# AlessioSam/LADiff

Hardware: AMD Instinct MI355X
Metric: motions/sec (196-frame, 50-step DDIM, bs128) (higher is better)
Workload: dtype f16x3+f32; 1 GPU; headline:ddim50_cfg7.5_b128_f196_c263_humanml3d; prompts_per_gpu=128, global_batch=128, frames=196, scheduler=ddim, denoising_steps=50, parallelism=dp1, loop=persistent pipeline kernel (16-row blocks x 86)

## Files before the change

### include/ladiff_hip_debug.h

```cpp
#ifndef LADIFF_HIP_DEBUG_H
#define LADIFF_HIP_DEBUG_H

#include "ladiff_hip.h"

#ifdef __cplusplus
extern "C" {
#endif

LADIFF_API int ladiff_debug_set_stage_waves(int waves_per_simd);
LADIFF_API int ladiff_debug_set_handoff(int tagged);
LADIFF_API int ladiff_debug_set_stage_plan(int v);
LADIFF_API int ladiff_debug_set_poll_pause(int mask, int len);
LADIFF_API int ladiff_debug_set_stage_delay(int mask, int len);
LADIFF_API int ladiff_debug_set_pacing(int eighths, int mask);
LADIFF_API int ladiff_debug_set_xcd_local(int on);
LADIFF_API int ladiff_debug_set_decoder_fusion(int on);
LADIFF_API int ladiff_debug_set_mlp_variant(int v);

LADIFF_API int ladiff_debug_set_loop_thresholds(int look_ahead_from, int small_upto);
LADIFF_API int ladiff_debug_set_graph_epoch_rule(int on);
LADIFF_API int ladiff_debug_graph_instantiations(void);

#ifdef LADIFF_STAMPS
LADIFF_API void ladiff_debug_set_stamps(unsigned long long* p);
LADIFF_API void ladiff_debug_set_sys_stamps(unsigned long long* p);
LADIFF_API void ladiff_debug_set_probe(int v);
#endif

#ifdef __cplusplus
}
#endif
#endif
```

### ladiff_amd/_lib.py

```python
import ctypes
import os
from ctypes import c_char_p, c_double, c_float, c_int, c_size_t, c_uint64, c_void_p

import numpy as np
import torch

_HERE = os.path.dirname(os.path.abspath(__file__))
LIB_PATH = os.path.join(_HERE, "libladiff_hip.so")

MAX_LATENTS = 8
MAX_FRAMES = 224
COEF_STRIDE = 8
COEF_K_NOISE, COEF_K_M = 5, 6
ACT = {"none": 0, "relu": 1, "gelu": 2, "silu": 3, "qgelu": 4, "lrelu": 5}


class LadiffHipError(RuntimeError):
    pass


SPLIT_MODES = ("f16x3", "bf16x3", "split")


def is_split(precision):
# ... 69 lines not shown
    "ladiff_reverse_status_offset_bytes": (c_size_t, [c_int, c_int, c_int, c_int]),
    "ladiff_debug_set_stage_plan": (c_int, [c_int]),
    "ladiff_debug_set_poll_pause": (c_int, [c_int, c_int]),
    "ladiff_debug_set_stage_delay": (c_int, [c_int, c_int]),
    "ladiff_debug_set_pacing": (c_int, [c_int, c_int]),
    "ladiff_debug_set_loop_thresholds": (c_int, [c_int, c_int]),
    "ladiff_debug_set_graph_epoch_rule": (c_int, [c_int]),
    "ladiff_debug_graph_instantiations": (c_int, []),
    "ladiff_sampler_set_fault": (c_int, [c_void_p, c_int, c_int]),
    "ladiff_sampler_set_noise_generator": (c_int, [c_void_p, c_uint64, ctypes.c_uint32, c_int]),
    "ladiff_noise_fill": (c_int, [c_uint64, ctypes.c_uint32, c_int, c_int, c_int, c_int, c_void_p, c_void_p]),
    "ladiff_reverse_workspace_bytes": (c_size_t, [c_int, c_int, c_int, c_int]),
    "ladiff_diffusion_reverse": (c_int, [c_void_p, c_void_p, c_void_p, c_uint64, c_void_p, c_void_p, c_void_p, c_void_p, c_void_p,
                                         c_void_p, c_void_p, c_void_p, c_float, c_float, c_int, c_int, c_int, c_int, c_int,
                                         c_void_p, c_void_p, c_size_t, c_int, c_void_p]),
    "ladiff_diffusion_reverse_prompts": (c_int, [c_void_p, c_void_p, c_void_p, c_uint64, c_void_p, c_void_p, c_void_p, c_void_p, c_void_p,
                                                 c_void_p, c_void_p, c_void_p, c_float, c_float, c_int, c_int, c_int, c_int, c_int,
                                                 c_void_p, c_void_p, c_size_t, c_int, c_void_p, c_void_p, c_void_p, c_int, c_void_p]),
    "ladiff_diffusion_reverse_multistep": (c_int, [c_void_p, c_void_p, c_void_p, c_uint64, c_void_p, c_void_p, c_void_p, c_void_p, c_void_p,
                                                   c_void_p, c_void_p, c_void_p, c_float, c_float, c_int, c_int, c_int, c_int, c_int,
                                                   c_void_p, c_void_p, c_size_t, c_int, c_void_p, c_void_p, c_void_p, c_int, c_void_p,
                                                   c_void_p]),
    "ladiff_diffusion_reverse_from": (c_int, [c_void_p, c_void_p, c_void_p, c_uint64, c_void_p, c_void_p, c_void_p, c_void_p, c_void_p,
                                              c_void_p, c_void_p, c_void_p, c_float, c_float, c_int, c_int, c_int, c_int, c_int,
                                              c_void_p, c_void_p, c_size_t, c_int, c_void_p, c_void_p, c_void_p, c_int, c_void_p,
                                              c_void_p, c_void_p, c_int, c_void_p]),
    "ladiff_diffusion_reverse_record": (c_int, [c_void_p, c_void_p, c_void_p, c_uint64, c_void_p, c_void_p, c_void_p, c_void_p, c_void_p,
                                                c_void_p, c_void_p, c_void_p, c_float, c_float, c_int, c_int, c_int, c_int, c_int,
                                                c_void_p, c_void_p, c_size_t, c_int, c_void_p, c_void_p, c_void_p, c_int, c_void_p,
                                                c_void_p, c_void_p, c_int, c_void_p, c_void_p, c_void_p]),
    "ladiff_noise_fill_prompts": (c_int, [c_void_p, c_void_p, c_int, c_int, c_int, c_int, c_void_p, c_void_p]),
    "ladiff_encoder_num_params": (c_int, []),
    "ladiff_encoder_param_name": (c_char_p, [c_int]),
    "ladiff_encoder_workspace_bytes": (c_size_t, [c_int, c_int, c_int, c_int]),
    "ladiff_vae_encode": (c_int, [c_void_p, c_void_p, c_void_p, c_void_p, c_void_p, c_void_p, c_int, c_int, c_int, c_int,
                                  c_void_p, c_void_p, c_void_p, c_void_p, c_size_t, c_void_p]),
    "ladiff_vae_encode_dvae": (c_int, [c_void_p, c_void_p, c_void_p, c_void_p, c_void_p, c_void_p, c_int, c_int, c_int, c_int,
                                       c_void_p, c_void_p, c_void_p, c_void_p, c_size_t, c_void_p, c_void_p, c_int, c_void_p]),
    "ladiff_vae_losses_workspace_bytes": (c_size_t, [c_int, c_int, c_int, c_int, c_int]),
    "ladiff_vae_losses": (c_int, [c_void_p, c_void_p, c_void_p, c_void_p, c_void_p, c_void_p, c_int, c_int, c_int, c_int, c_int,
                                  c_double, c_double, c_double, c_void_p, c_void_p, c_void_p, c_size_t, c_void_p]),
    "ladiff_denoiser_forward_timesteps_workspace_bytes": (c_size_t, [c_int, c_int]),
    "ladiff_denoiser_forward_timesteps": (c_int, [c_void_p, c_void_p, c_void_p, c_int, c_void_p, c_void_p, c_int, c_int, c_void_p, c_void_p,
                                                  c_void_p, c_size_t, c_void_p]),
    "ladiff_q_sample": (c_int, [c_void_p, c_void_p, c_void_p, c_int, c_void_p, c_int, c_uint64, ctypes.c_uint32, c_void_p, c_void_p, c_int,
                                c_int, c_void_p]),
    "ladiff_diffusion_losses_workspace_bytes": (c_size_t, [ctypes.c_int64]),
    "ladiff_diffusion_losses": (c_int, [c_void_p, c_void_p, ctypes.c_int64, c_double, c_void_p, c_void_p, c_void_p, c_size_t, c_void_p]),
    "ladiff_clip_num_params": (c_int, []),
    "ladiff_clip_param_name": (c_char_p, [c_int]),
    "ladiff_clip_workspace_bytes": (c_size_t, [c_int, c_int]),
    "ladiff_clip_text_encode": (c_int, [c_void_p, c_void_p, c_int, c_int, c_void_p, c_int, c_int, c_int, c_void_p, c_void_p,
                                        c_size_t, c_void_p]),
    "ladiff_clip_workspace_bytes_ragged": (c_size_t, [c_int, c_int]),
    "ladiff_clip_text_encode_ragged": (c_int, [c_void_p, c_void_p, c_int, c_int, c_void_p, c_int, c_int, c_int, c_void_p, c_void_p,
                                               c_void_p, c_int, c_void_p, c_void_p, c_size_t, c_void_p]),
    "ladiff_t2m_movement_num_params": (c_int, []),
    "ladiff_t2m_movement_param_name": (c_char_p, [c_int]),
    "ladiff_t2m_motion_num_params": (c_int, []),
    "ladiff_t2m_motion_param_name": (c_char_p, [c_int]),
    "ladiff_t2m_text_num_params": (c_int, []),
    "ladiff_t2m_text_param_name": (c_char_p, [c_int]),
    "ladiff_t2m_movement_workspace_bytes": (c_size_t, [c_int, c_int, c_int]),
    "ladiff_t2m_motion_workspace_bytes": (c_size_t, [c_int, c_int]),
    "ladiff_t2m_text_workspace_bytes": (c_size_t, [c_int, c_int]),
    "ladiff_t2m_movement_encode": (c_int, [c_void_p, c_void_p, c_int, c_int, c_int, c_int, c_void_p, c_void_p, c_size_t,
                                           c_void_p]),
    "ladiff_t2m_motion_encode": (c_int, [c_void_p, c_void_p, c_void_p, c_int, c_int, c_void_p, c_void_p, c_size_t, c_void_p]),
    "ladiff_t2m_text_encode": (c_int, [c_void_p, c_void_p, c_void_p, c_void_p, c_int, c_int, c_void_p, c_void_p, c_size_t,
                                       c_void_p]),
    "ladiff_feats2joints": (c_int, [c_void_p, c_void_p, c_void_p, c_int, c_int, c_int, c_int, c_void_p, c_void_p]),
    "ladiff_joints2feats": (c_int, [c_void_p, c_void_p, c_int, c_int, c_int, c_void_p, c_float, c_void_p, c_void_p, c_void_p, c_void_p]),
    "ladiff_joint_ape_ave": (c_int, [c_void_p, c_void_p, c_void_p, c_void_p, c_int, c_int, c_int, c_void_p, c_float, c_void_p, c_void_p,
                                     c_void_p]),
    "ladiff_joint_mr": (c_int, [c_void_p, c_void_p, c_void_p, c_int, c_int, c_int, c_void_p, c_void_p, c_void_p]),
    "ladiff_decoder_workspace_bytes": (c_size_t, [c_int, c_int, c_int, c_int]),
    "ladiff_vae_decode": (c_int, [c_void_p, c_void_p, c_void_p, c_void_p, c_void_p, c_int, c_int, c_int, c_int, c_void_p,
                                  c_void_p, c_size_t, c_void_p]),
    "ladiff_debug_set_stage_waves": (c_int, [c_int]),
    "ladiff_debug_set_handoff": (c_int, [c_int]),
    "ladiff_debug_set_xcd_local": (c_int, [c_int]),
    "ladiff_debug_set_decoder_fusion": (c_int, [c_int]),
    "ladiff_debug_set_mlp_variant": (c_int, [c_int]),
    "ladiff_reverse_plan": (c_int, [c_int, c_int, c_void_p, c_int, c_int, c_int, c_int, c_void_p, c_void_p]),
    "ladiff_decoder_graph_create": (c_int, [ctypes.POINTER(c_void_p)]),
    "ladiff_decoder_graph_destroy": (c_int, [c_void_p]),
    "ladiff_vae_decode_graphed": (c_int, [c_void_p, c_void_p, c_void_p, c_uint64, c_void_p, c_void_p, c_void_p, c_void_p, c_int, c_int, c_int,
                                          c_int, c_int, c_void_p, c_void_p, c_size_t, c_void_p]),
    "ladiff_vae_decode_ragged": (c_int, [c_void_p, c_void_p, c_void_p, c_void_p, c_void_p, c_void_p, c_int, c_int, c_int, c_int,
                                         c_int, c_void_p, c_void_p, c_size_t, c_void_p]),
    "ladiff_vae_decode_att_maps": (c_int, [c_void_p, c_void_p, c_void_p, c_void_p, c_void_p, c_void_p, c_int, c_int, c_int, c_int,
                                           c_int, c_void_p, c_void_p, c_void_p, c_size_t, c_void_p]),
}

EXPORTS = tuple(_SIGNATURES)
_lib = None
LIB_PATH_BF16 = os.path.join(_HERE, "libladiff_hip_bf16.so")


def select_split_format(fmt):
    global LIB_PATH, _lib
    if fmt not in ("fp16", "bf16"):
        raise ValueError(f'split format must be "fp16" or "bf16", got {fmt!r}')
    path = LIB_PATH_BF16 if fmt == "bf16" else os.path.join(_HERE, "libladiff_hip.so")
    if _lib is not None and path != LIB_PATH:
        raise LadiffHipError("select_split_format() after the library has been used: weight tables of the other format exist")
    LIB_PATH = path


def lib():
    global _lib
    if _lib is None:
        if not os.path.exists(LIB_PATH):
            raise LadiffHipError(f"{LIB_PATH} not found: build it with `python -m ladiff_amd.build` "
                                 "(the HIP library is the only implementation of this path; there is no CPU fallback)")
        cdll = ctypes.CDLL(LIB_PATH)
        for name, (res, args) in _SIGNATURES.items():
            fn = getattr(cdll, name)
            fn.restype, fn.argtypes = res, args
        _lib = cdll
    return _lib


def check(rc):
    if rc != 0:
        raise LadiffHipError(f"libladiff_hip: {lib().ladiff_error_string(rc).decode()} (code {rc})")


def ptr(t, dtype=torch.float32):
    if t is None:
        return None
    if not t.is_cuda:
        raise LadiffHipError("libladiff_hip works on GPU tensors only; got a CPU tensor (no CPU fallback exists)")
    if t.dtype != dtype:
        raise LadiffHipError(f"expected {dtype}, got {t.dtype}")
    if not t.is_contiguous():
        raise LadiffHipError("expected a contiguous tensor")
    return t.data_ptr()


def stream_ptr():
    return torch.cuda.current_stream().cuda_stream


def param_names(kind):
    l = lib()
    n = getattr(l, f"ladiff_{kind}_num_params")()
    return [getattr(l, f"ladiff_{kind}_param_name")(i).decode() for i in range(n)]


class WeightTable:
    _next_generation = 1

    def __init__(self, kind, tensors, n_names=None, no_split=(), pad_rows=None):
        self.generation = WeightTable._next_generation
        WeightTable._next_generation += 1
        names = param_names(kind)
        if n_names is not None:
            names = names[:n_names]
        self.no_split = set(no_split)
        self.pad_rows = dict(pad_rows or {})
        self.names = names
        self.tensors = []
        for n in names:
            if n not in tensors:
                raise LadiffHipError(f"missing weight {n}")
# ... 107 lines not shown
```

### ladiff_amd/csrc/api.hip

```cpp
#include <algorithm>
#include <cstdlib>
#include <cstring>
#include <vector>

#include "model.h"
#include "sampler.h"
#include "../../include/ladiff_hip_debug.h"

using namespace ladiff;

namespace {

inline hipStream_t S(ladiff_stream_t s) { return reinterpret_cast<hipStream_t>(s); }

bool all_set(const float* const* w, size_t n) {
    if (w == nullptr) return false;
    for (size_t i = 0; i < n; ++i)
        if (w[i] == nullptr) return false;
    return true;
}
template <class W>
bool load_weights(W& dst, const float* const* ptrs) {
    if (!all_set(ptrs, sizeof(W) / sizeof(const float*))) return false;
    std::memcpy(&dst, ptrs, sizeof(W));
// ... 206 lines not shown
}
int ladiff_init_latents(const float* noise, const int32_t* counts, float sigma, float* latents, int B, int T,
                        ladiff_stream_t stream) {
    LADIFF_CHECK_ARG(noise && latents && B > 0 && T > 0);
    return launch_init_latents(noise, counts, sigma, latents, B, T, S(stream));
}
int ladiff_init_latents_from(const float* z0, const float* noise, const uint64_t* seeds, const uint32_t* prompt_index, const int32_t* counts,
                             const float* coef, const int32_t* starts, int first_step, float* latents, int B, int T, ladiff_stream_t stream) {
    LADIFF_CHECK_ARG(z0 && coef && latents && B > 0 && T > 0 && first_step >= 0);
    LADIFF_CHECK_ARG(noise != nullptr || seeds != nullptr);
    LADIFF_CHECK_ARG(prompt_index == nullptr || seeds != nullptr);
    if ((reinterpret_cast<uintptr_t>(z0) & 15) || (reinterpret_cast<uintptr_t>(noise) & 15) || (reinterpret_cast<uintptr_t>(latents) & 15) ||
        (reinterpret_cast<uintptr_t>(seeds) & 7) || (reinterpret_cast<uintptr_t>(prompt_index) & 3) || (reinterpret_cast<uintptr_t>(starts) & 3))
        return LADIFF_ERR_SHAPE;
    const NoiseGen gen = noise == nullptr ? NoiseGen{0u, 0u, 0u, 1, reinterpret_cast<const unsigned long long*>(seeds), prompt_index}
                                          : NoiseGen{0u, 0u, 0u, 0};
    return launch_init_latents_from(z0, noise, gen, counts, coef, starts, first_step, latents, B, T, nullptr, S(stream));
}
int ladiff_finalize_latents(const float* latents, const int32_t* counts, float* z, int B, int T, ladiff_stream_t stream) {
    LADIFF_CHECK_ARG(latents && z && B > 0 && T > 0);
    return launch_finalize_latents(latents, counts, z, B, T, S(stream));
}

int ladiff_sampler_create(void** sampler) {
    LADIFF_CHECK_ARG(sampler);
    *sampler = new Sampler();
    return 0;
}
int ladiff_sampler_destroy(void* sampler) {
    Sampler* sp = reinterpret_cast<Sampler*>(sampler);
    if (sp == nullptr) return 0;
    (void)hipDeviceSynchronize();
    sp->drain_retired();
    if (sp->exec) (void)hipGraphExecDestroy(sp->exec);
    if (sp->setup) (void)hipGraphExecDestroy(sp->setup);
    if (sp->ev0) (void)hipEventDestroy(sp->ev0);
    if (sp->ev1) (void)hipEventDestroy(sp->ev1);
    for (hipEvent_t e : sp->wev) (void)hipEventDestroy(e);
    sp->cap.destroy();
    delete sp;
    return 0;
}

int ladiff_reverse_plan(int B, int T, const int32_t* h_counts, int masked, int loop_mode, int f16x3, int cfg, int* rows_per_block, int* n_blocks) {
    LADIFF_CHECK_ARG(B >= 1 && T >= 1 && T <= LADIFF_MAX_LATENTS && loop_mode >= 1 && loop_mode <= 3 && rows_per_block && n_blocks);
    if (!cfg && masked && h_counts == nullptr) return LADIFF_ERR_UNSUPPORTED;
    std::vector<unsigned char> plan;
    int mr = 2, nb = 0;
    choose_plan(B, T, h_counts, masked != 0, loop_mode, f16x3 != 0, plan, &mr, &nb, cfg != 0);
    *rows_per_block = 16 * mr; *n_blocks = nb;
    return 0;
}

int ladiff_debug_set_stage_waves(int waves_per_simd) {
    LADIFF_CHECK_ARG(waves_per_simd == 1 || waves_per_simd == 2);
    g_loop.waves16 = waves_per_simd;
    return 0;
}

int ladiff_debug_set_handoff(int tagged) {
    LADIFF_CHECK_ARG(tagged == 0 || tagged == 1);
    g_loop.handoff = tagged;
    return 0;
}

int ladiff_debug_set_mlp_variant(int v) {
#ifdef LADIFF_STAMPS
    LADIFF_CHECK_ARG((v >= 0 && v <= 3) || (v >= 11 && v <= 17) || (v >= 21 && v <= 26));
#else
    LADIFF_CHECK_ARG(v >= 0 && v <= 3);
#endif
    g_dec.mlp_variant = v;
    return 0;
}

int ladiff_debug_set_decoder_fusion(int on) {
    LADIFF_CHECK_ARG(on >= 0 && on <= 254 && (on & 3) != 3 && (on & 48) != 48);
    g_dec.post_off = (on & 128) ? 1 : 0;
    g_dec.out_cross = (on & 64) ? 0 : 1;
    g_dec.fused_mlp = on & 3;
    g_dec.small_rows_path = (on & 4) ? 0 : 1;
    g_dec.final_split = (on & 8) ? 0 : 1;
    g_dec.fused_attn = (on & 16) ? 0 : (on & 32) ? 2 : 1;
    return 0;
}

int ladiff_debug_set_stage_plan(int v) {
    LADIFF_CHECK_ARG(v >= 0 && v <= 1);
    g_loop.stage_plan = v;
    return 0;
}

int ladiff_debug_set_poll_pause(int mask, int len) {
    LADIFF_CHECK_ARG(mask >= 0 && mask <= 255 && len >= 0 && len <= 64);
    g_loop.poll_pause = mask | (len << 8);
    return 0;
}

int ladiff_debug_set_pacing(int eighths, int mask) {
    if (eighths == -1) { g_loop.pace = -1; return 0; }
    LADIFF_CHECK_ARG(eighths >= 0 && eighths <= 8 && mask >= 0 && mask <= 255);
    g_loop.pace = eighths | (mask << 8);
    return 0;
}

int ladiff_debug_set_stage_delay(int mask, int len) {
    LADIFF_CHECK_ARG(mask >= -1 && mask <= 255 && len >= 0 && len <= 64);
    g_loop.stage_delay = mask < 0 ? -1 : (mask | (len << 8));
    return 0;
}

int ladiff_debug_set_loop_thresholds(int look_ahead_from, int small_upto) {
    LADIFF_CHECK_ARG(look_ahead_from >= -1 && small_upto >= -1);
    g_loop.look_ahead_from = look_ahead_from;
    g_loop.small_upto = small_upto;
    return 0;
}

int ladiff_debug_set_graph_epoch_rule(int on) {
    LADIFF_CHECK_ARG(on == 0 || on == 1);
    g_graph_epoch_rule = on;
    return 0;
}

int ladiff_debug_graph_instantiations(void) { return g_graph_instantiations.load(); }

int ladiff_debug_set_xcd_local(int on) {
    LADIFF_CHECK_ARG(on >= 0 && on <= 2);
    g_loop.xcd_local = on;
    return 0;
}

int ladiff_sampler_set_loop(void* sampler, int mode) {
    Sampler* sp = reinterpret_cast<Sampler*>(sampler);
    LADIFF_CHECK_ARG(sp != nullptr && mode >= 0 && mode <= 3);
    sp->loop = mode != 0;
    sp->loop_mode = mode;
    return 0;
}

int ladiff_sampler_loop_ms(void* sampler, float* ms) {
    Sampler* sp = reinterpret_cast<Sampler*>(sampler);
    LADIFF_CHECK_ARG(sp != nullptr && ms != nullptr && sp->ev1 != nullptr);
    LADIFF_HIP(hipEventSynchronize(sp->ev1));
    LADIFF_HIP(hipEventElapsedTime(ms, sp->ev0, sp->ev1));
    return 0;
}

int ladiff_sampler_set_window_timing(void* sampler, int on) {
    Sampler* sp = reinterpret_cast<Sampler*>(sampler);
    LADIFF_CHECK_ARG(sp != nullptr);
    sp->time_windows = on != 0;
    return 0;
}

int ladiff_sampler_window_ms(void* sampler, float* loop_ms_sum, int* n_windows) {
    Sampler* sp = reinterpret_cast<Sampler*>(sampler);
    LADIFF_CHECK_ARG(sp != nullptr && loop_ms_sum != nullptr && n_windows != nullptr);
    float sum = 0.f;
    for (int i = 0; i < sp->n_windows; ++i) {
        float ms = 0.f;
        LADIFF_HIP(hipEventSynchronize(sp->wev[2 * i + 1]));
        LADIFF_HIP(hipEventElapsedTime(&ms, sp->wev[2 * i], sp->wev[2 * i + 1]));
        sum += ms;
    }
    *loop_ms_sum = sum; *n_windows = sp->n_windows;
// ... 476 lines not shown
```

### ladiff_amd/csrc/attention.hip

```cpp
#include "kernels.h"

namespace ladiff {

constexpr int SA_FMAX = LADIFF_MAX_FRAMES;
constexpr int SA_NKT = SA_FMAX / 32;

struct AttnGeom { int nheads, ld, koff, voff, out_ld, causal; };

__global__ __launch_bounds__(256) void dec_self_attn_kernel(const float* __restrict__ qkv, const int32_t* __restrict__ lengths,
                                                            const uint32_t* __restrict__ keybits, float* __restrict__ out,
                                                            int B, int F, int split_out, const AttnGeom g,
                                                            const int32_t* __restrict__ row_off, int shared_qkv) {
    __shared__ __attribute__((aligned(16))) float Ks[SA_FMAX * DH];
    __shared__ __attribute__((aligned(16))) float Vs[SA_FMAX * DH];
    const int tid = threadIdx.x, lane = tid & 63, wave = tid >> 6;
    const int b = blockIdx.y / g.nheads, h = blockIdx.y % g.nheads;
    int len = F;
    uint32_t kb[SA_NKT + 1];
    if (keybits != nullptr) {
        len = 1;
#pragma unroll
        for (int i = 0; i < SA_NKT; ++i) {
            kb[i] = keybits[(size_t)b * 8 + i];
            if (kb[i]) len = 32 * i + 32 - __builtin_clz(kb[i]);
// ... 46 lines not shown
            f32x16 acc;
#pragma unroll
            for (int i = 0; i < 16; ++i) acc[i] = 0.f;
            const int r = kt * 32 + q;
#pragma unroll
            for (int g8 = 0; g8 < 8; ++g8) {
                const f32x4 a = ld4(Ks + r * DH + ((((g8 << 1) + h2) ^ (r & 15)) << 2));
#pragma unroll
                for (int e = 0; e < 4; ++e) acc = __builtin_amdgcn_mfma_f32_32x32x2f32(a[e], qf[g8][e], acc, 0, 0, 0);
            }
#pragma unroll
            for (int i = 0; i < 16; ++i) {
                const int kin = (i & 3) + 8 * (i >> 2) + 4 * h2;
                const bool ok = ((kb[kt] >> kin) & 1u) && (!g.causal || kt * 32 + kin <= qrow);
                const float s = ok ? acc[i] : -INFINITY;
                acc[i] = s;
                m = fmaxf(m, s);
            }
            sT[kt] = acc;
        }
    }
    m = fmaxf(m, __shfl_xor(m, 32, 64));

    float l = 0.f;
#pragma unroll
    for (int kt = 0; kt < SA_NKT; ++kt) {
        if (kt < nkt) {
#pragma unroll
            for (int i = 0; i < 16; ++i) {
                const float pv = expf(sT[kt][i] - m);
                sT[kt][i] = pv;
                l += pv;
            }
        }
    }
    l += __shfl_xor(l, 32, 64);

    f32x16 o0, o1;
#pragma unroll
    for (int i = 0; i < 16; ++i) { o0[i] = 0.f; o1[i] = 0.f; }
#pragma unroll
    for (int kt = 0; kt < SA_NKT; ++kt) {
        if (kt < nkt) {
#pragma unroll
            for (int i = 0; i < 16; ++i) {
                const int key = kt * 32 + (i & 3) + 8 * (i >> 2) + 4 * h2;
                const float a0 = Vs[key * DH + q];
                const float a1 = Vs[key * DH + 32 + q];
                o0 = __builtin_amdgcn_mfma_f32_32x32x2f32(a0, sT[kt][i], o0, 0, 0, 0);
                o1 = __builtin_amdgcn_mfma_f32_32x32x2f32(a1, sT[kt][i], o1, 0, 0, 0);
            }
        }
    }

    if (qrow < F) {
        const float inv = 1.f / l;
        float* rowp = out + (row0 + qrow) * g.out_ld;
        const int c0 = h * DH + 4 * h2;
#pragma unroll
        for (int rg = 0; rg < 4; ++rg) {
            f32x4 v0, v1;
#pragma unroll
            for (int e = 0; e < 4; ++e) { v0[e] = o0[4 * rg + e] * inv; v1[e] = o1[4 * rg + e] * inv; }
            if (split_out) {
                store_split4(rowp, c0 + 8 * rg, v0);
                store_split4(rowp, c0 + 32 + 8 * rg, v1);
            } else {
                st4(rowp + c0 + 8 * rg, v0);
                st4(rowp + c0 + 32 + 8 * rg, v1);
            }
        }
    }
}


__device__ __forceinline__ void split8(const float (&v)[8], s16x8& hi, s16x8& lo) {
    split8(f32x4{v[0], v[1], v[2], v[3]}, f32x4{v[4], v[5], v[6], v[7]}, hi, lo);
}

template <int FM, int NT>
__global__ __launch_bounds__(NT, NT == 64 ? 2 : 1) void self_attn_split_kernel(const float* __restrict__ qkv, const int32_t* __restrict__ lengths,
                                                               const uint32_t* __restrict__ keybits, float* __restrict__ out,
                                                               int B, int F, int split_out, const AttnGeom g,
                                                               const int32_t* __restrict__ row_off, int shared_qkv) {
    constexpr int NKT = FM / 32, IT = FM * 16 / NT, VLD = FM + 8;
    static_assert(FM % 32 == 0 && (FM * 16) % NT == 0 && NT % 64 == 0 && (FM / 4) % (NT / 64) == 0 && NT / 64 >= FM / 32, "a wave per query tile");
    __shared__ __attribute__((aligned(16))) s16 Kp[2 * FM * DH];
    __shared__ __attribute__((aligned(16))) s16 Vt[2 * DH * VLD];
    s16* const Kh = Kp; s16* const Kl = Kp + FM * DH;
    s16* const Vth = Vt; s16* const Vtl = Vt + DH * VLD;
    float* const Vtmp = reinterpret_cast<float*>(Kp);
    const int tid = threadIdx.x, lane = tid & 63, wave = tid >> 6;
    const int b = blockIdx.x / g.nheads, h = blockIdx.x % g.nheads;
    int len = F;
    uint32_t kb[NKT + 1];
    if (keybits != nullptr) {
        len = 1;
#pragma unroll
        for (int i = 0; i < NKT; ++i) {
            kb[i] = keybits[(size_t)b * 8 + i];
            if (kb[i]) len = 32 * i + 32 - __builtin_clz(kb[i]);
        }
        len = len > F ? F : len;
    } else {
        len = lengths != nullptr ? lengths[b] : F;
        len = len < 1 ? 1 : (len > F ? F : len);
#pragma unroll
        for (int i = 0; i < NKT; ++i) kb[i] = len >= 32 * i + 32 ? 0xFFFFFFFFu : (len > 32 * i ? (1u << (len - 32 * i)) - 1u : 0u);
    }
    const int nkt = (len + 31) >> 5;
    size_t row0 = (size_t)b * F;
    if (row_off != nullptr) { row0 = row_off[b]; F = row_off[b + 1] - row_off[b]; }
    const size_t base = (shared_qkv ? (size_t)0 : row0) * g.ld + h * DH;

    const int qt = wave;
    const int q = lane & 31, h2 = lane >> 5;
    const int qrow = qt * 32 + q;

    s16x8 qh[4], ql[4];
#pragma unroll
    for (int ks = 0; ks < 4; ++ks) {
        float v[8] = {0.f, 0.f, 0.f, 0.f, 0.f, 0.f, 0.f, 0.f};
        if (qrow < F) {
            const f32x4 a = ld4(qkv + base + (size_t)qrow * g.ld + 16 * ks + 8 * h2);
            const f32x4 c = ld4(qkv + base + (size_t)qrow * g.ld + 16 * ks + 8 * h2 + 4);
#pragma unroll
            for (int e = 0; e < 4; ++e) { v[e] = a[e] * (0.125f * 1.4426950408889634f); v[4 + e] = c[e] * (0.125f * 1.4426950408889634f); }
        }
        split8(v, qh[ks], ql[ks]);
    }


    f32x4 kk[IT], vv[IT];
#pragma unroll
    for (int it = 0; it < IT; ++it) {
        const int id = tid + it * NT, r = id >> 4, c = id & 15;
        kk[it] = f32x4{0.f, 0.f, 0.f, 0.f}; vv[it] = kk[it];
        if (r < nkt * 32 && r < F) {
            const float* src = qkv + base + (size_t)r * g.ld + c * 4;
            kk[it] = ld4(src + g.koff);
            vv[it] = ld4(src + g.voff);
        }
    }
#pragma unroll
    for (int it = 0; it < IT; ++it) {
        const int id = tid + it * NT, r = id >> 4, c = id & 15;
        if (r < nkt * 32) st4(Vtmp + r * DH + c * 4, vv[it]);
    }
    __syncthreads();
    {
        const int d = tid & 63, kg = tid >> 6;
        for (int p = 0; p < FM / 4 / (NT / 64); ++p) {
            const int k0 = (p * (NT / 64) + kg) * 4;
            if (k0 < nkt * 32) {
                s16x4 hi, lo;
                split4(Vtmp[k0 * DH + d], Vtmp[(k0 + 1) * DH + d], Vtmp[(k0 + 2) * DH + d], Vtmp[(k0 + 3) * DH + d], hi, lo);
                *reinterpret_cast<s16x4*>(Vth + d * VLD + k0) = hi;
                *reinterpret_cast<s16x4*>(Vtl + d * VLD + k0) = lo;
            }
        }
    }
    __syncthreads();
#pragma unroll
    for (int it = 0; it < IT; ++it) {
        const int id = tid + it * NT, r = id >> 4, c = id & 15;
        if (r < nkt * 32) {
            s16x4 hi, lo;
            split4(kk[it], hi, lo);
            const int off = r * DH + ((((c >> 1) ^ ((r >> 1) & 7)) << 3) | ((c & 1) << 2));
            *reinterpret_cast<s16x4*>(Kh + off) = hi;
            *reinterpret_cast<s16x4*>(Kl + off) = lo;
        }
    }
    __syncthreads();

    if (qt * 32 >= F) return;
// ... 19 lines not shown
            if (kb[kt] == 0xFFFFFFFFu && !g.causal) {
#pragma unroll
                for (int i = 0; i < 16; ++i) m = fmaxf(m, acc[i]);
            } else {
#pragma unroll
                for (int i = 0; i < 16; ++i) {
                    const int kin = (i & 3) + 8 * (i >> 2) + 4 * h2;
                    const bool ok = ((kb[kt] >> kin) & 1u) && (!g.causal || kt * 32 + kin <= qrow);
                    const float s = ok ? acc[i] : -INFINITY;
                    acc[i] = s;
                    m = fmaxf(m, s);
                }
            }
            sT[kt] = acc;
        }
    }
    m = fmaxf(m, __shfl_xor(m, 32, 64));

    float l = 0.f;
#pragma unroll
    for (int kt = 0; kt < NKT; ++kt) {
        if (kt < nkt) {
#pragma unroll
            for (int i = 0; i < 16; ++i) {
                const float pv = __builtin_amdgcn_exp2f(sT[kt][i] - m);
                sT[kt][i] = pv;
                l += pv;
            }
        }
    }
    l += __shfl_xor(l, 32, 64);

    f32x16 o0, o1;
#pragma unroll
    for (int i = 0; i < 16; ++i) { o0[i] = 0.f; o1[i] = 0.f; }
#pragma unroll
    for (int kt = 0; kt < NKT; ++kt) {
        if (kt < nkt) {
#pragma unroll
            for (int mm = 0; mm < 2; ++mm) {
                float pv[8];
#pragma unroll
                for (int j = 0; j < 8; ++j) pv[j] = sT[kt][8 * mm + j];
                s16x8 ph, pl;
                split8(pv, ph, pl);
                const int k1 = 32 * kt + 16 * mm + 4 * h2;
#pragma unroll
                for (int t = 0; t < 2; ++t) {
                    const int voff = (32 * t + q) * VLD + k1;
                    const s16x4 h_a = *reinterpret_cast<const s16x4*>(Vth + voff), h_b = *reinterpret_cast<const s16x4*>(Vth + voff + 8);
                    const s16x4 l_a = *reinterpret_cast<const s16x4*>(Vtl + voff), l_b = *reinterpret_cast<const s16x4*>(Vtl + voff + 8);
                    const s16x8 vh = {h_a[0], h_a[1], h_a[2], h_a[3], h_b[0], h_b[1], h_b[2], h_b[3]};
                    const s16x8 vl = {l_a[0], l_a[1], l_a[2], l_a[3], l_b[0], l_b[1], l_b[2], l_b[3]};
                    f32x16& o = t == 0 ? o0 : o1;
                    o = MFMA32_S16(vl, ph, o, 0, 0, 0);
                    o = MFMA32_S16(vh, pl, o, 0, 0, 0);
                    o = MFMA32_S16(vh, ph, o, 0, 0, 0);
                }
            }
        }
    }

    if (qrow < F) {
        const float inv = 1.f / l;
        float* rowp = out + (row0 + qrow) * g.out_ld;
        const int c0 = h * DH + 4 * h2;
#pragma unroll
        for (int rg = 0; rg < 4; ++rg) {
            f32x4 v0, v1;
#pragma unroll
            for (int e = 0; e < 4; ++e) { v0[e] = o0[4 * rg + e] * inv; v1[e] = o1[4 * rg + e] * inv; }
            if (split_out) {
                store_split4(rowp, c0 + 8 * rg, v0);
                store_split4(rowp, c0 + 32 + 8 * rg, v1);
            } else {
                st4(rowp + c0 + 8 * rg, v0);
                st4(rowp + c0 + 32 + 8 * rg, v1);
            }
        }
    }
}

int launch_self_attention_split(const float* qkv, const int32_t* lengths, const uint32_t* keybits, float* out, int B, int F,
                                 int nheads, int causal, int split_out, hipStream_t s, const int32_t* row_off, int shared_qkv) {
    if (F > SA_FMAX || F < 1 || nheads < 1) return LADIFF_ERR_SHAPE;
    if (B == 0) return 0;
    const int W = nheads * DH;
    const AttnGeom g{nheads, 3 * W, W, 2 * W, W, causal};
    if (F <= 32) hipLaunchKernelGGL((self_attn_split_kernel<32, 64>), dim3(B * nheads), dim3(64), 0, s, qkv, lengths, keybits, out, B, F, split_out, g, row_off, shared_qkv);
    else hipLaunchKernelGGL((self_attn_split_kernel<SA_FMAX, 512>), dim3(B * nheads), dim3(512), 0, s, qkv, lengths, keybits, out, B, F, split_out, g, row_off, shared_qkv);
    LADIFF_LAUNCH_CHECK();
    return 0;
}

int launch_self_attention(const float* qkv, const int32_t* lengths, const uint32_t* keybits, float* out, int B, int F, int nheads,
                          int causal, int split_out, hipStream_t s, const int32_t* row_off) {
    if (F > SA_FMAX || F < 1 || nheads < 1) return LADIFF_ERR_SHAPE;
    if (B == 0) return 0;
    const int W = nheads * DH;
    const AttnGeom g{nheads, 3 * W, W, 2 * W, W, causal};
    const int nqt = (F + 31) / 32;
    hipLaunchKernelGGL(dec_self_attn_kernel, dim3((nqt + 3) / 4, B * nheads), dim3(256), 0, s, qkv, lengths, keybits, out, B, F,
                       split_out, g, row_off, 0);
    LADIFF_LAUNCH_CHECK();
    return 0;
}

int launch_decoder_self_attention(const float* qkv, const int32_t* lengths, const uint32_t* keybits, float* out, int B, int F,
                                  int split_out, hipStream_t s, const int32_t* row_off, int shared_qkv) {
    if (F > SA_FMAX || F < 1) return LADIFF_ERR_SHAPE;
    if (lengths == nullptr && keybits == nullptr) return LADIFF_ERR_ARG;
    if (B == 0) return 0;
    const AttnGeom g{H, 3 * D, D, 2 * D, D, 0};
    const int nqt = (F + 31) / 32;
    hipLaunchKernelGGL(dec_self_attn_kernel, dim3((nqt + 3) / 4, B * H), dim3(256), 0, s, qkv, lengths, keybits, out, B, F,
                       split_out, g, row_off, shared_qkv);
    LADIFF_LAUNCH_CHECK();
    return 0;
}

template <int T>
__global__ __launch_bounds__(256) void dec_cross_attn_kernel(const float* __restrict__ q, const float* __restrict__ kv,
                                                             const int32_t* __restrict__ counts, float* __restrict__ out,
                                                             int B, int F, int M, int split_out) {
    const int row = blockIdx.x * 4 + (threadIdx.x >> 6);
    if (row >= M) return;
    const int c = (threadIdx.x & 63) * 4;
    const int b = row / F;
    int nv = counts ? counts[b] : T;
    nv = nv < 1 ? 1 : (nv > T ? T : nv);
    f32x4 qv = ld4(q + (size_t)row * D + c);
    float s[T];
    float m = -INFINITY;
#pragma unroll
    for (int j = 0; j < T; ++j) {
        const f32x4 kk = ld4(kv + ((size_t)j * B + b) * 512 + c);
        float d = (qv[0] * 0.125f) * kk[0] + (qv[1] * 0.125f) * kk[1] + (qv[2] * 0.125f) * kk[2] + (qv[3] * 0.125f) * kk[3];
        d = row16_sum(d);
        s[j] = j < nv ? d : -INFINITY;
        m = fmaxf(m, s[j]);
    }
    float l = 0.f;
    f32x4 o = {0.f, 0.f, 0.f, 0.f};
#pragma unroll
    for (int j = 0; j < T; ++j) {
        const float pv = expf(s[j] - m);
        l += pv;
        const f32x4 vv = ld4(kv + ((size_t)j * B + b) * 512 + 256 + c);
#pragma unroll
        for (int e = 0; e < 4; ++e) o[e] += pv * vv[e];
    }
    const float inv = 1.f / l;
#pragma unroll
    for (int e = 0; e < 4; ++e) o[e] *= inv;
    if (split_out) store_split4(out + (size_t)row * D, c, o);
    else st4(out + (size_t)row * D + c, o);
}

int launch_decoder_cross_attention(const float* q, const float* kv, const int32_t* counts, float* out, int B, int F,
                                   int T, int split_out, hipStream_t s) {
    const int M = B * F;
    if (M == 0) return 0;
    const dim3 grid((M + 3) / 4), block(256);
#define LADIFF_CA_CASE(TT) \
    case TT: hipLaunchKernelGGL(dec_cross_attn_kernel<TT>, grid, block, 0, s, q, kv, counts, out, B, F, M, split_out); break;
    switch (T) {
        LADIFF_CA_CASE(1) LADIFF_CA_CASE(2) LADIFF_CA_CASE(3) LADIFF_CA_CASE(4)
        LADIFF_CA_CASE(5) LADIFF_CA_CASE(6) LADIFF_CA_CASE(7) LADIFF_CA_CASE(8)
        default: return LADIFF_ERR_SHAPE;
    }
#undef LADIFF_CA_CASE
    LADIFF_LAUNCH_CHECK();
    return 0;
// ... 82 lines not shown
```

### ladiff_amd/csrc/common.h

```cpp
#pragma once
#include <hip/hip_runtime.h>
#include <stdint.h>

#include "weights.h"

namespace ladiff {

constexpr float LN_EPS = 1e-5f;
constexpr int CLIP_MAX_LAYERS = LADIFF_CLIP_MAX_LAYERS;
constexpr int CLIP_MAX_POSITIONS = LADIFF_CLIP_MAX_POSITIONS;

typedef float f32x4 __attribute__((ext_vector_type(4)));
typedef float f32x16 __attribute__((ext_vector_type(16)));

#define LADIFF_CHECK_ARG(cond) \
    do { if (!(cond)) return LADIFF_ERR_ARG; } while (0)
#define LADIFF_HIP(expr) \
    do { hipError_t e_ = (expr); if (e_ != hipSuccess) return (int)e_; } while (0)
#define LADIFF_TRY(expr) \
    do { int r_ = (expr); if (r_ != 0) return r_; } while (0)
#define LADIFF_LAUNCH_CHECK() LADIFF_HIP(hipGetLastError())

__device__ __forceinline__ float erf_as(float x) {
    const float ax = fabsf(x);
    const float t = __builtin_amdgcn_rcpf(fmaf(0.3275911f, ax, 1.f));
    float q = fmaf(t, 1.061405429f, -1.453152027f);
    q = fmaf(t, q, 1.421413741f);
    q = fmaf(t, q, -0.284496736f);
    q = fmaf(t, q, 0.254829592f);
    const float e = __builtin_amdgcn_exp2f(-1.4426950408889634f * ax * ax);
    return copysignf(fmaf(-q * t, e, 1.f), x);
}
__device__ __forceinline__ float gelu_erf(float v) { return 0.5f * v * (1.f + erf_as(v * 0.70710678118654752440f)); }
typedef float f32x2 __attribute__((ext_vector_type(2)));
__device__ __forceinline__ f32x2 gelu_erf2(f32x2 v) {
    const f32x2 x = v * 0.70710678118654752440f;
    const f32x2 ax = f32x2{fabsf(x[0]), fabsf(x[1])};
    const f32x2 d = __builtin_elementwise_fma(f32x2{0.3275911f, 0.3275911f}, ax, f32x2{1.f, 1.f});
    const f32x2 t = f32x2{__builtin_amdgcn_rcpf(d[0]), __builtin_amdgcn_rcpf(d[1])};
    f32x2 q = __builtin_elementwise_fma(t, f32x2{1.061405429f, 1.061405429f}, f32x2{-1.453152027f, -1.453152027f});
    q = __builtin_elementwise_fma(t, q, f32x2{1.421413741f, 1.421413741f});
    q = __builtin_elementwise_fma(t, q, f32x2{-0.284496736f, -0.284496736f});
    q = __builtin_elementwise_fma(t, q, f32x2{0.254829592f, 0.254829592f});
    const f32x2 a2 = (-1.4426950408889634f * ax) * ax;
    const f32x2 e = f32x2{__builtin_amdgcn_exp2f(a2[0]), __builtin_amdgcn_exp2f(a2[1])};
    const f32x2 r = __builtin_elementwise_fma(-q * t, e, f32x2{1.f, 1.f});
    const f32x2 er = f32x2{copysignf(r[0], x[0]), copysignf(r[1], x[1])};
    return (0.5f * v) * (1.f + er);
}

enum Act : int { ACT_NONE = 0, ACT_RELU = 1, ACT_GELU = 2, ACT_SILU = 3, ACT_QGELU = 4, ACT_LRELU = 5 };

__device__ __forceinline__ float act_apply(float v, int act) {
    switch (act) {
        case ACT_RELU: return fmaxf(v, 0.f);
        case ACT_GELU: return gelu_erf(v);
        case ACT_SILU: return v / (1.f + expf(-v));
        case ACT_QGELU: return v / (1.f + expf(-1.702f * v));
        case ACT_LRELU: return v > 0.f ? v : 0.2f * v;
        default: return v;
    }
}

template <int ACT>
__device__ __forceinline__ float act_c(float v) {
    if constexpr (ACT == ACT_RELU) return fmaxf(v, 0.f);
    else if constexpr (ACT == ACT_GELU) return gelu_erf(v);
    else if constexpr (ACT == ACT_SILU) return v / (1.f + expf(-v));
    else if constexpr (ACT == ACT_QGELU) return v / (1.f + expf(-1.702f * v));
    else if constexpr (ACT == ACT_LRELU) return v > 0.f ? v : 0.2f * v;
    else return v;
}
template <int V> struct IntC { static constexpr int value = V; };
template <class F>
__device__ __forceinline__ void act_dispatch(int act, F&& f) {
    switch (act) {
        case ACT_RELU: f(IntC<ACT_RELU>{}); break;
        case ACT_GELU: f(IntC<ACT_GELU>{}); break;
        case ACT_SILU: f(IntC<ACT_SILU>{}); break;
        case ACT_QGELU: f(IntC<ACT_QGELU>{}); break;
        case ACT_LRELU: f(IntC<ACT_LRELU>{}); break;
        default: f(IntC<ACT_NONE>{}); break;
    }
}

__device__ __forceinline__ float silu(float v) { return v / (1.f + expf(-v)); }

template <int WIDTH>
__device__ __forceinline__ float group_sum(float v) {
#pragma unroll
    for (int o = WIDTH / 2; o > 0; o >>= 1) v += __shfl_xor(v, o, 64);
    return v;
}
template <int WIDTH>
__device__ __forceinline__ float group_max(float v) {
#pragma unroll
    for (int o = WIDTH / 2; o > 0; o >>= 1) v = fmaxf(v, __shfl_xor(v, o, 64));
    return v;
}

template <int CTRL, int ROW_MASK = 0xF>
__device__ __forceinline__ float dpp_add(float v) {
    return v + __builtin_bit_cast(float, __builtin_amdgcn_update_dpp(0, __builtin_bit_cast(int, v), CTRL, ROW_MASK, 0xF, true));
}
__device__ __forceinline__ float row16_sum(float v) {
    v = dpp_add<0xB1>(v);
    v = dpp_add<0x4E>(v);
    v = dpp_add<0x141>(v);
    v = dpp_add<0x140>(v);
    return v;
}
__device__ __forceinline__ float wave_sum(float v) {
    v = row16_sum(v);
    v = dpp_add<0x142, 0xA>(v);
    v = dpp_add<0x143, 0xC>(v);
    return __builtin_bit_cast(float, __builtin_amdgcn_readlane(__builtin_bit_cast(int, v), 63));
}
template <int CTRL, int ROW_MASK = 0xF>
__device__ __forceinline__ float dpp_max(float v) {
    return fmaxf(v, __builtin_bit_cast(float, __builtin_amdgcn_update_dpp(0, __builtin_bit_cast(int, v), CTRL, ROW_MASK, 0xF, true)));
}
template <int CTRL, int ROW_MASK = 0xF>
__device__ __forceinline__ uint32_t dpp_add_u32(uint32_t v) {
    return v + (uint32_t)__builtin_amdgcn_update_dpp(0, (int)v, CTRL, ROW_MASK, 0xF, true);
}
__device__ __forceinline__ float wave_max_nonneg(float v) {
    v = dpp_max<0xB1>(v);
    v = dpp_max<0x4E>(v);
    v = dpp_max<0x141>(v);
    v = dpp_max<0x140>(v);
    v = dpp_max<0x142, 0xA>(v);
    v = dpp_max<0x143, 0xC>(v);
    return __builtin_bit_cast(float, __builtin_amdgcn_readlane(__builtin_bit_cast(int, v), 63));
}
__device__ __forceinline__ uint32_t wave_sum_u32(uint32_t v) {
    v = dpp_add_u32<0xB1>(v);
    v = dpp_add_u32<0x4E>(v);
    v = dpp_add_u32<0x141>(v);
    v = dpp_add_u32<0x140>(v);
    v = dpp_add_u32<0x142, 0xA>(v);
    v = dpp_add_u32<0x143, 0xC>(v);
    return (uint32_t)__builtin_amdgcn_readlane((int)v, 63);
}

#ifndef LADIFF_SPLIT_BF16
typedef _Float16 s16;
#define MFMA16_S16 __builtin_amdgcn_mfma_f32_16x16x32_f16
#define MFMA32_S16 __builtin_amdgcn_mfma_f32_32x32x16_f16
__device__ __forceinline__ s16 s16_of(float v) { return (_Float16)__builtin_amdgcn_fmed3f(v, -65504.f, 65504.f); }
typedef s16 s16x2 __attribute__((ext_vector_type(2)));
__device__ __forceinline__ void split2(float a, float b, s16x2& hi, s16x2& lo) {
    hi = __builtin_bit_cast(s16x2, __builtin_amdgcn_cvt_pkrtz(a, b));
    lo = __builtin_bit_cast(s16x2, __builtin_amdgcn_cvt_pkrtz(a - (float)hi[0], b - (float)hi[1]));
}
#else
typedef __bf16 s16;
#define MFMA16_S16 __builtin_amdgcn_mfma_f32_16x16x32_bf16
#define MFMA32_S16 __builtin_amdgcn_mfma_f32_32x32x16_bf16
__device__ __forceinline__ s16 s16_of(float v) { return (__bf16)v; }
typedef s16 s16x2 __attribute__((ext_vector_type(2)));
__device__ __forceinline__ void split2(float a, float b, s16x2& hi, s16x2& lo) {
    hi[0] = (__bf16)a; hi[1] = (__bf16)b;
    lo[0] = (__bf16)(a - (float)hi[0]); lo[1] = (__bf16)(b - (float)hi[1]);
}
#endif
typedef s16 s16x8 __attribute__((ext_vector_type(8)));
typedef s16 s16x4 __attribute__((ext_vector_type(4)));
__device__ __forceinline__ void split4(float a, float b, float c, float d, s16x4& hi, s16x4& lo) {
    s16x2 h0, l0, h1, l1;
// ... 49 lines not shown
```

### ladiff_amd/csrc/dec_post.hip

```cpp
#include <mutex>
#include "model.h"
#include "tile_mma.h"

namespace ladiff {

namespace {

constexpr int PST_NS = 8;
constexpr int PST_GRP = 4;
constexpr int PST_STAGE = 16384;
constexpr int PST_NV = 11;
constexpr int PST_LDS = PST_NS * PST_STAGE + FF * 4 + PST_NV * D * 4;

typedef unsigned u32x4_p __attribute__((ext_vector_type(4)));

__device__ __forceinline__ int pi_row(int p) { const int j = p >> 4, n = p & 15; return 32 * (j >> 1) + 8 * (n >> 2) + 4 * (j & 1) + (n & 3); }

template <int N> __device__ __forceinline__ void wait_vm() { asm volatile("s_waitcnt vmcnt(%0)" ::"n"(N) : "memory"); }
template <int OFF>
__device__ __forceinline__ void fetch16(u32x4_p& v, unsigned addr) {
    asm volatile("ds_read_b128 %0, %1 offset:%2" : "=v"(v) : "v"(addr), "n"(OFF) : "memory");
}
template <int N>
__device__ __forceinline__ void wait_lgkm(u32x4_p& a, u32x4_p& b, u32x4_p& c, u32x4_p& d) {
    asm volatile("s_waitcnt lgkmcnt(%4)" : "+v"(a), "+v"(b), "+v"(c), "+v"(d) : "n"(N));
}
__device__ __forceinline__ s16x8 as_s16(const u32x4_p v) { return __builtin_bit_cast(s16x8, v); }

}

__global__ __launch_bounds__(256) void dec_post_gu_kernel(float* guws, size_t gu_layer, int T) {
    __shared__ float us[32 * 257];
    const int tid = threadIdx.x, HT = H * T;
    float* g = guws + blockIdx.y * gu_layer + (size_t)blockIdx.x * HT * 2 * D;
    for (int hj = 0; hj < HT; ++hj) us[hj * 257 + tid] = g[(size_t)(2 * hj + 1) * D + tid];
    __syncthreads();
    const int lane = tid & 63, n = lane & 15, fk = lane >> 4;
    for (int i = 0; i < HT; ++i) {
        const int q = 4 * i + (tid >> 6), jj = q / T, e = q - jj * T;
        const int col = 32 * (jj >> 1) + 8 * (n >> 2) + 4 * (jj & 1) + (n & 3);
        g[(size_t)(2 * i + 1) * D + tid] = us[(fk * T + e) * 257 + col];
    }
}

template <int TT>
__global__ __launch_bounds__(512, 2) void dec_post_kernel(const DecPostArgs p) {
    constexpr int NW = 8, NT = 64 * NW, PPW = 16 / NW;
    extern __shared__ __attribute__((aligned(1024))) char lds[];
    float* const b1s = reinterpret_cast<float*>(lds + PST_NS * PST_STAGE);
    float* const prm = b1s + FF;
    const int tid = threadIdx.x, lane = tid & 63;
    const int wave = __builtin_amdgcn_readfirstlane(tid >> 6);
    const int frow = lane & 15, fk = lane >> 4;
    constexpr int T = TT;
    const int M = p.M;

    const int t = blockIdx.x * NW + wave;
    int b = 0, f0 = 0, len = p.F, ntiles;
    if (p.row_off == nullptr) {
        const int tps = (p.F + 15) >> 4;
        ntiles = p.B * tps;
        b = t / tps; f0 = 16 * (t - b * tps);
    } else {
        int base = 0;
        for (int i0 = 0; i0 < p.B; i0 += 64) {
            const int i = i0 + lane;
            const int nt = i < p.B ? (p.row_off[i + 1] - p.row_off[i] + 15) >> 4 : 0;
            int incl = nt;
#pragma unroll
            for (int o = 1; o < 64; o <<= 1) { const int up = __shfl_up(incl, o, 64); if (lane >= o) incl += up; }
            incl += base;
            const unsigned long long hit = __ballot(t >= incl - nt && t < incl);
            if (hit != 0ull) {
                const int src = __ffsll((long long)hit) - 1;
                b = i0 + src; f0 = 16 * (t - __shfl(incl - nt, src, 64));
            }
            base = __shfl(incl, 63, 64);
        }
        ntiles = base;
    }
    if (blockIdx.x * NW >= ntiles) return;
    const bool tile_ok = t < ntiles;
    b = __builtin_amdgcn_readfirstlane(tile_ok ? b : 0);
    f0 = __builtin_amdgcn_readfirstlane(tile_ok ? f0 : 0);
    int srow = b * p.F;
    if (p.row_off != nullptr) { srow = p.row_off[b]; len = p.row_off[b + 1] - srow; }
    int nrows = len - f0 < 16 ? len - f0 : 16;
    nrows = tile_ok ? nrows : 0;
    const int row0 = srow + f0;
    const int myrow = nrows > 0 ? row0 + (frow < nrows ? frow : nrows - 1) : M - 1;

    s16x8 xh[8], xl[8];
    {
        const char* xr = reinterpret_cast<const char*>(p.att) + (size_t)myrow * 1024 + fk * 16;
#pragma unroll
        for (int s = 0; s < 8; ++s) {
            xh[s] = *reinterpret_cast<const s16x8*>(xr + (s >> 1) * 256 + (s & 1) * 64);
            xl[s] = *reinterpret_cast<const s16x8*>(xr + (s >> 1) * 256 + (s & 1) * 64 + 128);
        }
    }
    f32x4 hacc[8], oacc[16];
#pragma unroll
    for (int jj = 0; jj < 16; ++jj) oacc[jj] = ld4(p.x0 + (size_t)myrow * D + 32 * (jj >> 1) + 8 * fk + 4 * (jj & 1));
    float cv[8];
    {
        const float* cb = p.cc + (size_t)b * (H * T) + fk * T;
#pragma unroll
        for (int e = 0; e < 8; ++e) cv[e] = e < T ? cb[e < T ? e : 0] : 0.f;
    }
    int nv = p.counts != nullptr ? p.counts[b] : T;
    nv = nv > T ? T : nv;
    for (int i = tid; i < FF / 4; i += NT) st4(b1s + 4 * i, ld4(p.b1 + 4 * i));
    for (int i = tid; i < PST_NV * D / 4; i += NT) {
        const int which = i / (D / 4), c4 = i % (D / 4);
        const float* src = which == 0 ? p.b2 : which == 1 ? p.g3 : which == 2 ? p.be3 : which == 3 ? p.g4 : which == 4 ? p.be4
                         : which == 5 ? p.bo : which == 6 ? p.g1 : which == 7 ? p.be1 : which == 8 ? p.bo_c : which == 9 ? p.g2 : p.be2;
        if (src != nullptr) st4(prm + 4 * i, ld4(src + 4 * c4));
    }

    const int cs = (lane & 7) ^ ((lane >> 4) & 3) ^ (4 * (wave & 1));
    const int koff = (cs < 4 ? cs * 4 : 32 + (cs - 4) * 4);
    int src[PPW];
#pragma unroll
    for (int i = 0; i < PPW; ++i) src[i] = pi_row(8 * (wave + NW * i) + (lane >> 3));
    char* const dma_dst = lds + (8 * wave) * 128;
    auto issue = [&](auto woc, int hs, auto uc, auto slotc, auto ic) __attribute__((always_inline)) {
        constexpr bool wo = decltype(woc)::value != 0;
        constexpr int u = decltype(uc)::value, slot = decltype(slotc)::value, i = decltype(ic)::value;
        const float* base; int ldw, n0, kb, half;
        if constexpr (wo) { constexpr int c = u >> 1; base = p.wo; ldw = D; n0 = 128 * (u & 1); kb = c >> 1; half = c & 1; }
        else if constexpr (u < 8) { base = p.w1; ldw = D; n0 = 128 * hs; kb = u >> 1; half = u & 1; }
        else { constexpr int v = u - 8, c = v >> 1; base = p.w2; ldw = FF; n0 = 128 * (v & 1); kb = 2 * hs + (c >> 1); half = c & 1; }
        const float* s0 = base + (size_t)(n0 + src[i]) * ldw + kb * 64 + half * 16 + koff;
        __builtin_amdgcn_global_load_lds(s0, (__attribute__((address_space(3))) void*)(dma_dst + slot * PST_STAGE + 8 * NW * i * 128), 16, 0, 0);
    };

    const int sw = (frow >> 1) & 7;
    const unsigned rd_hi = lds_addr(lds) + frow * 128 + ((fk ^ sw) << 4);
    const unsigned rd_lo = lds_addr(lds) + frow * 128 + (((4 + fk) ^ sw) << 4);
    const unsigned rd_hi2 = rd_hi + 4 * PST_STAGE, rd_lo2 = rd_lo + 4 * PST_STAGE;

    s16x8 hh[4], hl[4];

    u32x4_p wt[4][2];
    auto fetch_tile = [&](auto slotc, auto jc) __attribute__((always_inline)) {
        constexpr int slot = decltype(slotc)::value, j = decltype(jc)::value;
        const unsigned ah = slot < 4 ? rd_hi : rd_hi2, al = slot < 4 ? rd_lo : rd_lo2;
        constexpr int so = (slot & 3) * PST_STAGE;
        fetch16<so + j * 2048>(wt[j & 3][0], ah); fetch16<so + j * 2048>(wt[j & 3][1], al);
    };
    auto stage_mma = [&](auto slotc, auto& acc, auto j0c, const s16x8 bh, const s16x8 bl, auto&& between, auto&& next) __attribute__((always_inline)) {
        constexpr int slot = decltype(slotc)::value, J0 = decltype(j0c)::value;
        static_for<8>([&](auto jc) {
            constexpr int j = decltype(jc)::value, cur = j & 3;
            next(jc);
            asm volatile("s_waitcnt lgkmcnt(4)" : "+v"(wt[cur][0]), "+v"(wt[cur][1]));
            __builtin_amdgcn_sched_barrier(0);
            acc[J0 + j] = MFMA16_S16(as_s16(wt[cur][0]), bl, acc[J0 + j], 0, 0, 0);
            __builtin_amdgcn_sched_barrier(0);
            if constexpr (j + 3 < 8) fetch_tile(slotc, IntC<j + 3>{});
            else fetch_tile(IntC<(slot + 1) % PST_NS>{}, IntC<j + 3 - 8>{});
            __builtin_amdgcn_sched_barrier(0);
            acc[J0 + j] = MFMA16_S16(as_s16(wt[cur][1]), bh, acc[J0 + j], 0, 0, 0);
            acc[J0 + j] = MFMA16_S16(as_s16(wt[cur][0]), bh, acc[J0 + j], 0, 0, 0);
            __builtin_amdgcn_sched_barrier(0);
            if constexpr (j & 1) between(IntC<j / 2>{});
        });
    };

    auto landed = [&]() __attribute__((always_inline)) {
        wait_vm<0>();
        __builtin_amdgcn_s_barrier();
    };
    auto stage = [&](auto woc, int hs, auto uc) __attribute__((always_inline)) {
        constexpr bool wo = decltype(woc)::value != 0;
        constexpr int u = decltype(uc)::value, slot = u % PST_NS, r = u % PST_GRP;
        auto batch_piece = [&](auto aheadc, auto halfc) __attribute__((always_inline)) {
            constexpr int ua = u + decltype(aheadc)::value, ut = ua % 16, slot_t = ua % PST_NS;
            if constexpr (wo && ua < 16) issue(IntC<1>{}, 0, IntC<ut>{}, IntC<slot_t>{}, halfc);
            else if constexpr (wo) issue(IntC<0>{}, 0, IntC<ut>{}, IntC<slot_t>{}, halfc);
            else issue(IntC<0>{}, (hs + (ua >= 16 ? 1 : 0)) & 7, IntC<ut>{}, IntC<slot_t>{}, halfc);
        };
        auto between = [&](auto gc) __attribute__((always_inline)) {
            constexpr int g = decltype(gc)::value;
            if constexpr (r == 3 && g >= 2) batch_piece(IntC<5>{}, IntC<g - 2>{});
            else if constexpr (r == 0 && g < 2) batch_piece(IntC<5>{}, IntC<g>{});
// ... 248 lines not shown
```

### ladiff_amd/csrc/decoder.hip

```cpp
#include "model.h"

namespace ladiff {

#ifdef LADIFF_STAMPS
#define DEC_CUT() do { if (dec_cut >= 0 && ++dec_launched >= dec_cut) { dec_done = true; return 0; } } while (0)
#define DEC_STEP(step) do { LADIFF_TRY(step); if (dec_done) return 0; } while (0)
#else
#define DEC_CUT() do { } while (0)
#define DEC_STEP(step) LADIFF_TRY(step)
#endif

DecSwitchAtoms g_dec;

int vae_decode(const DecoderW& w, const DecoderW* wsp, const float* z, const int32_t* lengths, const int32_t* counts,
               const int32_t* row_off, int R, int B, int F, int T, int C, float* feats, float* ws, size_t ws_floats, hipStream_t s, const DecSwitches& sw,
               float* att_maps) {
    if (F < 1 || F > LADIFF_MAX_FRAMES || T < 1 || T > LADIFF_MAX_LATENTS || C < 1) return LADIFF_ERR_SHAPE;
    const bool ragged = row_off != nullptr;
    if (ragged && (R < 0 || (size_t)R > (size_t)B * F)) return LADIFF_ERR_SHAPE;
    const int M = ragged ? R : B * F;
    DecWs a = dec_layout(ws, B, (size_t)M, T);
    if (ws_floats < a.total) return LADIFF_ERR_WORKSPACE;
    if (M == 0) return 0;
#ifdef LADIFF_STAMPS
    const char* dec_cut_env = getenv("LADIFF_DEC_CUT");
    const int dec_cut = dec_cut_env ? atoi(dec_cut_env) : -1;
    int dec_launched = 0; bool dec_done = false;
    if (dec_cut == 0) return 0;
#endif
    const bool sp = wsp != nullptr;
    DecSwitches swr = sw;
    if (att_maps != nullptr) swr.out_cross = 0;
    const DecRoute rt = dec_route(sp, M, swr, dec_mlp_min_rows());
    const Seq c{sp, M, s};
    const DecoderW& wm = mfma_table(w, wsp);
    Twin P[4], SK[NSKIP];
    pair_up(sp, a.P, a.Ps, P); pair_up(sp, a.SK, a.SKs, SK);
    const Twin pex = pair(sp, a.pex, a.pexs), att_x = operand_only(sp, a.att), hid_x = operand_only(sp, a.hid);
    float *qkv = a.qkv, *att = a.att, *hid = a.hid, *kv = a.kv, *guws = a.guws, *qkv0 = a.qkv0;

    {
        GemmArgs g[NL];
        DecCrossPrepBatch pb;
        for (int l = 0; l < NL; ++l) {
            const DecLayerW& L = w.layer[l];
            g[l] = lin(z, D, L.cross_attn.in_w + (size_t)D * D, L.cross_attn.in_b + D, kv + l * a.kv_layer, 2 * D, T * B, 2 * D, D);
            pb.kv[l] = kv + l * a.kv_layer; pb.wq[l] = L.cross_attn.in_w; pb.bq[l] = L.cross_attn.in_b; pb.wo[l] = L.cross_attn.out_w;
            pb.gu[l] = guws + l * a.gu_layer;
        }
        LADIFF_TRY(launch_gemm_batch(g, NL, s)); DEC_CUT();
        LADIFF_TRY(launch_decoder_cross_prep(pb, NL, B, T, s)); DEC_CUT();
        if (rt.post) { LADIFF_TRY(launch_dec_post_gu(guws, a.gu_layer, NL, B, T, s)); DEC_CUT(); }
    }

    auto krs = [&](Twin x, int K, const LinearW& W, Twin y, int ldy, int N, int act, const float* res, int rows) -> int {
        KrArgs g = proj_kr(Seq{sp, rows, s}, x, K, W, y, ldy, N, act, res);
        g.ldres = D;
        return launch_gemm_kr(g, s);
    };
    int l = 0; DecLayerW L; Twin cur = P[0];

    auto skip_concat = [&]() -> int {
        const LinearW sk = mixed(w.skip[l - NSKIP - 1], wm.skip[l - NSKIP - 1]);
        LADIFF_TRY(rt.small ? skip_rowln(c, cur, SK[NL - 1 - l], sk, P[3]) : skip_gemm(c, cur, SK[NL - 1 - l], sk, P[3])); DEC_CUT();
        cur = P[3];
        return 0;
    };

    auto self_attention = [&]() -> int {
        const LinearW in = in_proj(L.self_attn);
        const bool shared = l == 0; const Twin q = {shared ? qkv0 : qkv, nullptr};
        if (shared) {
            LADIFF_TRY(launch_broadcast_pe(w.query_pe, 1, F, pex.f, pex.s, s)); DEC_CUT();
            if (rt.small) { LADIFF_TRY(krs(pex, D, in, q, 3 * D, 3 * D, ACT_NONE, nullptr, F)); DEC_CUT(); }
            else { LADIFF_TRY(launch_gemm(proj(Seq{sp, F, s}, pex, D, in, q, 3 * D, 3 * D), s)); DEC_CUT(); }
        } else if (rt.fused_attn) {
            LADIFF_TRY(launch_dec_qkv_attn(cur.s, in.w, in.b, lengths, row_off, att, B, F, 1, s)); DEC_CUT();
            return 0;
        } else if (rt.small) { LADIFF_TRY(krs(cur, D, in, q, 3 * D, 3 * D, ACT_NONE, nullptr, M)); DEC_CUT(); }
        else { LADIFF_TRY(launch_gemm(proj(c, cur, D, in, q, 3 * D, 3 * D), s)); DEC_CUT(); }
        if (sp) { LADIFF_TRY(launch_self_attention_split(q.f, lengths, nullptr, att, B, F, H, 0, 1, s, row_off, shared)); DEC_CUT(); }
        else { LADIFF_TRY(launch_decoder_self_attention(q.f, lengths, nullptr, att, B, F, 0, s, row_off, shared)); DEC_CUT(); }
        return 0;
    };

    auto out_proj_cross_attention = [&]() -> int {
        const LinearW out = out_proj(L.self_attn); float* gu = guws + l * a.gu_layer;
        if (rt.out_cross) {
            LADIFF_TRY(launch_decoder_out_cross(att, cur.f, out.w, out.b, L.norm1.g, L.norm1.b, L.cross_attn.out_b, L.norm2.g, L.norm2.b,
                                                counts, B, F, T, gu, P[2].f, P[2].s, s, row_off)); DEC_CUT();
            return 0;
        }
        const Twin r1 = {P[1].f, nullptr};
        if (rt.small) { LADIFF_TRY(krs(att_x, D, out, r1, D, D, ACT_NONE, cur.f, M)); DEC_CUT(); }
        else if (sp) { LADIFF_TRY(launch_gemm(proj(c, att_x, D, out, r1, D, D, ACT_NONE, cur.f), s)); DEC_CUT(); }
        else { LADIFF_TRY(gemm_ln(c, att_x, D, out, cur.f, L.norm1, nullptr, r1, true)); DEC_CUT(); }
        const NormW n1_late = sp ? L.norm1 : NormW{nullptr, nullptr};
        if (att_maps != nullptr) {
            LADIFF_TRY(launch_decoder_cross_maps(P[1].f, counts, lengths, B, F, T, gu, att_maps + (size_t)l * B * F * T, s, row_off, n1_late.g,
                                                 n1_late.b)); DEC_CUT();
        }
        LADIFF_TRY(launch_decoder_cross_apply(P[1].f, L.cross_attn.out_b, L.norm2.g, L.norm2.b, counts, B, F, T, gu, P[2].f, P[2].s, s, row_off,
                                              n1_late.g, n1_late.b)); DEC_CUT();
        return 0;
    };

    auto feed_forward = [&](Twin dst) -> int {
        const NormW* fin = l == NL - 1 ? &w.norm : nullptr;
        if (rt.fused_mlp) {
            LADIFF_TRY(launch_dec_mlp(P[2].s, P[2].f, L.lin1.w, L.lin1.b, L.lin2.w, L.lin2.b, L.norm3.g, L.norm3.b, fin ? fin->g : nullptr,
                                      fin ? fin->b : nullptr, dst.f, dst.s, M, s, sw.mlp_variant)); DEC_CUT();
        } else if (rt.small) {
            LADIFF_TRY(krs(P[2], D, L.lin1, hid_x, FF, FF, ACT_GELU, nullptr, M)); DEC_CUT();
            LADIFF_TRY(krs(hid_x, FF, LinearW{L.lin2.w, nullptr}, Twin{qkv, nullptr}, D, D, ACT_NONE, nullptr, M)); DEC_CUT();
            RedArgs r = red(c, qkv, 4, L.lin2.b, P[2].f, &L.norm3, dst);
            if (fin) { r.g2 = fin->g; r.b2 = fin->b; }
            LADIFF_TRY(launch_reduce_rows(r, s));
        } else {
            LADIFF_TRY(launch_gemm(proj(c, P[2], D, L.lin1, hid_x, FF, FF, ACT_GELU), s)); DEC_CUT();
            LADIFF_TRY(gemm_ln(c, hid_x, FF, L.lin2, P[2].f, L.norm3, fin, dst, true)); DEC_CUT();
        }
        return 0;
    };

    auto post_attention = [&](Twin dst) -> int {
        const LinearW out = out_proj(L.self_attn); const float* gu = guws + l * a.gu_layer;
        const NormW* fin = l == NL - 1 ? &w.norm : nullptr;
        const DecPostArgs pa{att, cur.f, out.w, out.b, L.norm1.g, L.norm1.b, gu, gu + (size_t)B * H * T * 2 * D, L.cross_attn.out_b, L.norm2.g,
                             L.norm2.b, counts, row_off, L.lin1.w, L.lin1.b, L.lin2.w, L.lin2.b, L.norm3.g, L.norm3.b,
                             fin ? fin->g : nullptr, fin ? fin->b : nullptr, dst.f, dst.s, B, F, T, M};
        LADIFF_TRY(launch_dec_post(pa, s)); DEC_CUT();
        return 0;
    };

    if (ragged) { LADIFF_TRY(launch_broadcast_pe_ragged(w.query_pe, row_off, B, F, F, P[0].f, P[0].s, a.row_out, s)); DEC_CUT(); }
    else { LADIFF_TRY(launch_broadcast_pe(w.query_pe, B, F, P[0].f, P[0].s, s)); DEC_CUT(); }
    for (l = 0; l < NL; ++l) {
        L = mixed(w.layer[l], wm.layer[l]);
        if (l > NSKIP) DEC_STEP(skip_concat());
        DEC_STEP(self_attention());
        const Twin dst = l < NSKIP ? SK[l] : P[0];
        if (rt.post) DEC_STEP(post_attention(dst));
        else {
            DEC_STEP(out_proj_cross_attention());
            DEC_STEP(feed_forward(dst));
        }
        cur = dst;
    }
    if (rt.final_split) {
        const int Np = (C + 127) / 128 * 128;
        if ((size_t)M * Np > a.hid_floats || (size_t)Np * (D + 1) > a.qkv_floats) return LADIFF_ERR_SHAPE;
        float* wpad = qkv; float* bpad = qkv + (size_t)Np * D;
        LADIFF_TRY(launch_pad_rows(wm.final_layer.w, w.final_layer.b, wpad, bpad, C, Np, s)); DEC_CUT();
        LADIFF_TRY(launch_gemm(proj(c, cur, D, LinearW{wpad, bpad}, Twin{hid, nullptr}, Np, Np), s)); DEC_CUT();
        return launch_scatter_feats(hid, Np, C, M, F, ragged ? nullptr : lengths, ragged ? a.row_out : nullptr, feats, s);
    }
    GemmArgs g = lin(cur.f, D, w.final_layer, feats, C, M, C, D);
    if (ragged) g.row_map = a.row_out;
    else { g.row_len = lengths; g.rows_per_item = F; }
    return launch_gemm(g, s);
}

}
```

### ladiff_amd/csrc/denoiser.hip

```cpp
#include "model.h"

namespace ladiff {

static std::vector<std::string> block_prefixes(const char* root) {
    std::vector<std::string> v;
    for (int i = 0; i < NSKIP; ++i) v.push_back(std::string(root) + ".input_blocks." + std::to_string(i));
    v.push_back(std::string(root) + ".middle_block");
    for (int i = 0; i < NSKIP; ++i) v.push_back(std::string(root) + ".output_blocks." + std::to_string(i));
    return v;
}
static void wb(std::vector<std::string>& v, const std::string& p) { v.push_back(p + ".weight"); v.push_back(p + ".bias"); }
static void mha_names(std::vector<std::string>& v, const std::string& p) {
    v.push_back(p + ".in_proj_weight"); v.push_back(p + ".in_proj_bias"); wb(v, p + ".out_proj");
}
static void styl_names(std::vector<std::string>& v, const std::string& p) {
    wb(v, p + ".emb_layers.1"); wb(v, p + ".norm"); wb(v, p + ".out_layers.2");
}

const std::vector<std::string>& denoiser_param_names() {
    static const std::vector<std::string> names = [] {
        std::vector<std::string> v;
        wb(v, "time_embedding.linear_1"); wb(v, "time_embedding.linear_2"); wb(v, "emb_proj.1");
        v.push_back("query_pos.pe"); v.push_back("mem_pos.pe");
        wb(v, "encoder.norm");
// ... 27 lines not shown
        return v;
    }();
    return names;
}

const std::vector<std::string>& encoder_param_names() {
    static const std::vector<std::string> names = [] {
        std::vector<std::string> v;
        v.push_back("global_motion_token"); v.push_back("query_pos_encoder.pe");
        for (const auto& p : block_prefixes("encoder")) {
            mha_names(v, p + ".self_attn");
            wb(v, p + ".linear1"); wb(v, p + ".linear2");
            wb(v, p + ".norm1"); wb(v, p + ".norm2");
        }
        for (int i = 0; i < NSKIP; ++i) wb(v, "encoder.linear_blocks." + std::to_string(i));
        wb(v, "encoder.norm"); wb(v, "skel_embedding");
        return v;
    }();
    return names;
}

int denoiser_time_tables(const DenoiserW& w, const float* sinus, int n, float* tables, float* ws, size_t ws_floats,
                         hipStream_t s) {
    const DenTimeWs t = den_time_layout(ws, n);
    if (ws_floats < t.total) return LADIFF_ERR_WORKSPACE;
    float *h1 = t.h1, *temb = t.temb, *semb = t.semb;
    LADIFF_TRY(launch_gemm(lin(sinus, TEXT_DIM, w.time1, h1, D, n, D, TEXT_DIM, ACT_SILU), s));
    LADIFF_TRY(launch_gemm(lin(h1, D, w.time2, temb, D, n, D, D), s));
    LADIFF_TRY(launch_silu(temb, semb, (size_t)n * D, s));
    for (int l = 0; l < NL; ++l) {
        const DenLayerW& L = w.layer[l];
        float* base = tables + (size_t)l * DEN_LAYER_STRIDE;
        LADIFF_TRY(launch_gemm(lin(semb, D, L.ca_proj.emb, base + DEN_OFF_CA_MOD, DEN_STEP_STRIDE, n, 2 * D, D), s));
        LADIFF_TRY(launch_gemm(lin(semb, D, L.ffn_proj.emb, base + DEN_OFF_FFN_MOD, DEN_STEP_STRIDE, n, 2 * D, D), s));
        LinearW kvw{L.sa_attn.in_w + (size_t)D * D, L.sa_attn.in_b + D};
        LADIFF_TRY(launch_gemm(lin(temb, D, kvw, base + DEN_OFF_TIME_KV, DEN_STEP_STRIDE, n, 2 * D, D), s));
    }
    return 0;
}

static int denoiser_text_cache_general(const DenoiserW& w, const float* text, int B2, int N, float* cache, float* ws, size_t ws_floats,
                                       hipStream_t s) {
    const int R = B2 * N;
    const DenTextWs t = den_text_layout(ws, B2, 1, N);
    if (ws_floats < t.total) return LADIFF_ERR_WORKSPACE;
    const DenTextCache c = den_text_cache_layout(cache, B2, 1, N);
    float *rl = t.rl, *tn = t.tn, *key = t.key, *val = t.val, *tproj = c.tproj, *tkv = c.tkv, *catt = c.catt;
    LADIFF_TRY(launch_relu(text, rl, (size_t)R * TEXT_DIM, s));
    LADIFF_TRY(launch_gemm(lin(rl, TEXT_DIM, w.emb_proj, tproj, D, R, D, TEXT_DIM), s));
    for (int l = 0; l < NL; ++l) {
        const DenLayerW& L = w.layer[l];
        LinearW kvw{L.sa_attn.in_w + (size_t)D * D, L.sa_attn.in_b + D};
        LADIFF_TRY(launch_gemm(lin(tproj, D, kvw, tkv + (size_t)l * R * 2 * D, 2 * D, R, 2 * D, D), s));
        LADIFF_TRY(launch_layernorm(tproj, L.ca_text_norm.g, L.ca_text_norm.b, tn, R, s));
        LADIFF_TRY(launch_gemm(lin(tn, D, L.ca_key, key, D, R, D, D), s));
        LADIFF_TRY(launch_gemm(lin(tn, D, L.ca_value, val, D, R, D, D), s));
        LADIFF_TRY(launch_lca_kv(key, val, B2, N, catt + (size_t)l * B2 * H * DH * DH, s));
    }
    return 0;
}

int denoiser_text_static(const DenoiserW& w, const float* text, int B2, float* cache, float* ws, size_t ws_floats, hipStream_t s) {
    const DenTextWs t = den_text_layout(ws, B2, 0, 1);
    if (ws_floats < t.total) return LADIFF_ERR_WORKSPACE;
    const DenTextCache c = den_text_cache_layout(cache, B2, 0, 1);
    float *rl = t.rl, *tn = t.tn, *tproj = c.tproj, *tkv = c.tkv, *nval = c.nval;
    LADIFF_TRY(launch_relu(text, rl, (size_t)B2 * TEXT_DIM, s));
    LADIFF_TRY(launch_gemm(lin(rl, TEXT_DIM, w.emb_proj, tproj, D, B2, D, TEXT_DIM), s));
    GemmArgs kv[NL], val[NL];
    RowBatch ln;
    for (int l = 0; l < NL; ++l) {
        const DenLayerW& L = w.layer[l];
        LinearW kvw{L.sa_attn.in_w + (size_t)D * D, L.sa_attn.in_b + D};
        kv[l] = lin(tproj, D, kvw, tkv + (size_t)l * B2 * 2 * D, 2 * D, B2, 2 * D, D);
        ln.a[l] = tproj; ln.g[l] = L.ca_text_norm.g; ln.b[l] = L.ca_text_norm.b; ln.y[l] = tn + (size_t)l * B2 * D;
        val[l] = lin(tn + (size_t)l * B2 * D, D, L.ca_value, nval + (size_t)l * B2 * D, D, B2, D, D);
        val[l].ln_g = L.ca_proj.norm.g; val[l].ln_b = L.ca_proj.norm.b;
    }
    LADIFF_TRY(launch_gemm_batch(kv, NL, s));
    LADIFF_TRY(launch_layernorm_batch(ln, NL, B2, s));
    return launch_gemm_batch(val, NL, s);
}

int denoiser_ctab(const DenoiserW& w, const float* tables_lo, int n, float* cache, int B2, float* u, size_t u_floats, hipStream_t s,
                  const DenoiserW* wsp) {
    const int R = B2 + 1;
    const size_t u_all = den_text_layout(nullptr, B2, n, 1).u_floats;
    if (u_floats < u_all / NL) return LADIFF_ERR_WORKSPACE;
    const DenTextCache c = den_text_cache_layout(cache, B2, n, 1);
    const float* nval = c.nval;
    float* ctab = c.ctab;
    if (u_floats >= u_all) {
        RowBatch rb;
        GemmArgs g[NL];
        for (int l = 0; l < NL; ++l) {
            const DenLayerW& L = w.layer[l];
            float* ul = u + (size_t)l * n * R * D;
            rb.a[l] = nval + (size_t)l * B2 * D; rb.g[l] = L.ca_proj.norm.b;
            rb.b[l] = tables_lo + (size_t)l * DEN_LAYER_STRIDE + DEN_OFF_CA_MOD; rb.y[l] = ul;
            g[l] = lin(ul, D, L.ca_proj.out, ctab + (size_t)l * n * R * D, D, n * R, D, D);
            if (wsp != nullptr) { g[l].W = wsp->layer[l].ca_proj.out.w; g[l].split = 1; }
        }
        LADIFF_TRY(launch_ca_table_input_batch(rb, NL, DEN_STEP_STRIDE, n, B2, s, wsp != nullptr ? 1 : 0));
        return launch_gemm_batch(g, NL, s);
    }
    for (int l = 0; l < NL; ++l) {
        const DenLayerW& L = w.layer[l];
        LADIFF_TRY(launch_ca_table_input(nval + (size_t)l * B2 * D, L.ca_proj.norm.b, tables_lo + (size_t)l * DEN_LAYER_STRIDE + DEN_OFF_CA_MOD,
                                         DEN_STEP_STRIDE, n, B2, u, s));
        LADIFF_TRY(launch_gemm(lin(u, D, L.ca_proj.out, ctab + (size_t)l * n * R * D, D, n * R, D, D), s));
    }
    return 0;
}

int denoiser_text_cache(const DenoiserW& w, const float* text, int B2, const float* tables, int n, float* cache,
                        float* ws, size_t ws_floats, hipStream_t s, int ntxt) {
    if (ntxt > 1) return denoiser_text_cache_general(w, text, B2, ntxt, cache, ws, ws_floats, s);
    const DenTextWs t = den_text_layout(ws, B2, n, 1);
    if (ws_floats < t.total) return LADIFF_ERR_WORKSPACE;
    LADIFF_TRY(denoiser_text_static(w, text, B2, cache, ws, ws_floats, s));
    return denoiser_ctab(w, tables, n, cache, B2, t.u, t.u_floats, s, nullptr);
}

int linear_cross_attention(const DenoiserW& w, int layer, const float* x, const float* xf, const float* emb, const int32_t* counts,
                           int B, int T, int N, float* out, float* ws, size_t ws_floats, hipStream_t s) {
    if (layer < 0 || layer >= NL || T < 1 || T > LADIFF_MAX_LATENTS || N < 1) return LADIFF_ERR_SHAPE;
    const LcaWs a = lca_layout(ws, B, T, N);
    if (ws_floats < a.total) return LADIFF_ERR_WORKSPACE;
    const DenLayerW& L = w.layer[layer];
    const int R = B * N, M = B * T;
    float *tn = a.tn, *key = a.key, *val = a.val, *catt = a.catt, *xn = a.xn, *q = a.q, *semb = a.semb, *mod = a.mod;
    LADIFF_TRY(launch_layernorm(xf, L.ca_text_norm.g, L.ca_text_norm.b, tn, R, s));
    LADIFF_TRY(launch_gemm(lin(tn, D, L.ca_key, key, D, R, D, D), s));
    LADIFF_TRY(launch_gemm(lin(tn, D, L.ca_value, val, D, R, D, D), s));
    LADIFF_TRY(launch_lca_kv(key, val, B, N, catt, s));
    LADIFF_TRY(launch_layernorm(x, L.ca_norm.g, L.ca_norm.b, xn, M, s));
    LADIFF_TRY(launch_gemm(lin(xn, D, L.ca_query, q, D, M, D, D), s));
    LADIFF_TRY(launch_silu(emb, semb, (size_t)B * D, s));
    LADIFF_TRY(launch_gemm(lin(semb, D, L.ca_proj.emb, mod, 2 * D, B, 2 * D, D), s));
    LADIFF_TRY(launch_lca_apply(q, catt, counts, B, 0, B, T, mod, 0, 2 * D, nullptr, L.ca_proj.norm.g, L.ca_proj.norm.b, xn, s));
    GemmArgs g = lin(xn, D, L.ca_proj.out, out, D, M, D, D);
    g.res = x; g.ldres = D;
    return launch_gemm(g, s);
}


int denoiser_forward(const DenoiserW& w, const DenoiserW* wsp, const float* tables, const int32_t* d_step, const float* cache,
                     int n_steps, const float* sample, int Bs, int dup, int T, const int32_t* counts, float* eps, float* ws,
                     size_t ws_floats, hipStream_t s, int b_lo, int b_n, int loop_mode, int ntxt, const int32_t* d_base,
                     const float* dctab) {
    const int B2 = Bs * dup;
    const bool per_sample = d_step == nullptr;
    if (per_sample && (dctab == nullptr || ntxt != 1 || loop_mode)) return LADIFF_ERR_ARG;
    if (b_n < 0) { b_lo = 0; b_n = B2; }
    const int M = b_n * T;
    if (T < 1 || T > LADIFF_MAX_LATENTS || b_lo < 0 || b_lo + b_n > B2) return LADIFF_ERR_SHAPE;
    if (M == 0) return 0;
    DenForwardWs a = den_forward_layout(ws, (size_t)M);
    if (ws_floats < a.total) return LADIFF_ERR_WORKSPACE;
    eps += (size_t)b_lo * T * D;
    const bool sp = wsp != nullptr;
    const Seq c{sp, M, s};
    const DenoiserW& wm = mfma_table(w, wsp);
    Twin P[4], SK[NSKIP];
    pair_up(sp, a.P, a.Ps, P); pair_up(sp, a.SK, a.SKs, SK);
    float *qkv = a.qkv, *att = a.att, *hid = a.hid, *part = a.part;
    const Twin hid_x = operand_only(sp, hid);
    const float* tkv = den_cache_tkv(cache, B2, ntxt);
    const float* ctab = den_cache_ctab(cache, B2, ntxt);
    const int R = B2 + 1;
    auto gemm = [&](Twin x, int K, const LinearW& W, Twin y, int ldy, int N, int act = ACT_NONE, const float* res = nullptr) {
        return launch_gemm_kr(proj_kr(c, x, K, W, y, ldy, N, act, res), s);
    };

    if (!loop_mode) LADIFF_TRY(launch_add_pe(sample, w.query_pe, Bs, b_lo, b_n, T, P[0].f, P[0].s, s));
    Twin cur = P[0];
    for (int l = 0; l < NL; ++l) {
        const DenLayerW L = mixed(w.layer[l], wm.layer[l]);
        const LinearW in = in_proj(L.sa_attn), out = out_proj(L.sa_attn);
        const float* tl = tables + (size_t)l * DEN_LAYER_STRIDE;
        if (l > NSKIP) {
            const LinearW sk = mixed(w.skip[l - NSKIP - 1], wm.skip[l - NSKIP - 1]);
            if (sp) LADIFF_TRY(skip_rowln(c, cur, SK[NL - 1 - l], sk, P[3]));
            else {
                LADIFF_TRY(skip_kr(c, cur, SK[NL - 1 - l], sk, part));
                LADIFF_TRY(launch_reduce_rows(red(c, part, 2, sk.b, nullptr, nullptr, P[3]), s));
// ... 71 lines not shown
```

### ladiff_amd/csrc/gemm.h

```cpp
#pragma once
#include "common.h"

namespace ladiff {

struct GemmArgs {
    const float* A = nullptr;  int lda = 0;
    const float* A2 = nullptr; int lda2 = 0;
    int K1 = 0;
    const float* W = nullptr;  int ldw = 0;
    const float* bias = nullptr;
    float* Y = nullptr;        int ldy = 0;
    float* Ys = nullptr;
    int split = 0;
    int M = 0, N = 0, K = 0;
    int act = ACT_NONE;
    const float* res = nullptr; int ldres = 0;
    const float* ln_g = nullptr; const float* ln_b = nullptr;
    const float* ln2_g = nullptr; const float* ln2_b = nullptr;
    const float* mod = nullptr;
    const int32_t* d_step = nullptr; int mod_stride = 0;
    int post_act = ACT_NONE;
    const int32_t* row_len = nullptr; int rows_per_item = 0;
    const int32_t* row_map = nullptr;
    int ksplit = 1; size_t plane = 0;
};

int launch_gemm(const GemmArgs& a, hipStream_t stream);
constexpr int GEMM_BATCH_MAX = 9;
struct GemmBatch { GemmArgs a[GEMM_BATCH_MAX]; };
int launch_gemm_batch(const GemmArgs* list, int n, hipStream_t stream);
int launch_gemm_big_batch(const GemmBatch& b, int n, hipStream_t stream);
bool gemm_big_supported(const GemmArgs& a);
int launch_gemm_big(const GemmArgs& a, hipStream_t stream);

}
```

### ladiff_amd/csrc/gemm.hip

```cpp
#include "gemm.h"

namespace ladiff {

constexpr int BK = 32;

template <int MT> struct Mfma;
template <> struct Mfma<32> {
    typedef f32x16 Acc;
    static constexpr int REGS = 16;
    static constexpr int KGROUP = 8;
    __device__ static __forceinline__ Acc zero() { Acc a; for (int i = 0; i < 16; ++i) a[i] = 0.f; return a; }
    __device__ static __forceinline__ Acc mma(float a, float b, Acc c) {
        return __builtin_amdgcn_mfma_f32_32x32x2f32(a, b, c, 0, 0, 0);
    }
    __device__ static __forceinline__ int lane_row(int lane) { return lane & 31; }
    __device__ static __forceinline__ int lane_kgrp(int lane) { return lane >> 5; }
    __device__ static __forceinline__ int acc_row(int lane, int r) { return (r & 3) + 8 * (r >> 2) + 4 * (lane >> 5); }
    __device__ static __forceinline__ int acc_col(int lane) { return lane & 31; }
};
template <> struct Mfma<16> {
    typedef f32x4 Acc;
    static constexpr int REGS = 4;
    static constexpr int KGROUP = 16;
    __device__ static __forceinline__ Acc zero() { Acc a; for (int i = 0; i < 4; ++i) a[i] = 0.f; return a; }
// ... 180 lines not shown
            if (WN > 1) {
                __syncthreads();
#pragma unroll
                for (int i = 0; i < RM; ++i)
#pragma unroll
                    for (int r = 0; r < MM::REGS; ++r) {
                        float s = 0.f;
#pragma unroll
                        for (int w = 0; w < WN; ++w) s += red2[(wm * TMW + i * MT + MM::acc_row(lane, r)) * WN + w];
                        rstd[i][r] = rsqrtf(s * (1.f / 256.f) + LN_EPS);
                    }
            }
#pragma unroll
            for (int j = 0; j < RN; ++j) {
                const int gc = acol_base + j * MT;
                const float gg = g[gc], bb = b[gc];
#pragma unroll
                for (int i = 0; i < RM; ++i)
#pragma unroll
                    for (int r = 0; r < MM::REGS; ++r)
                        acc[i][j][r] = (acc[i][j][r] - mean[i][r]) * rstd[i][r] * gg + bb;
            }
        }
        if (mod != nullptr) {
#pragma unroll
            for (int j = 0; j < RN; ++j) {
                const int gc = acol_base + j * MT;
                const float sc = 1.f + mod[gc], sh = mod[256 + gc];
#pragma unroll
                for (int i = 0; i < RM; ++i)
#pragma unroll
                    for (int r = 0; r < MM::REGS; ++r) acc[i][j][r] = acc[i][j][r] * sc + sh;
            }
        }
    }

#pragma unroll
    for (int i = 0; i < RM; ++i)
#pragma unroll
        for (int r = 0; r < MM::REGS; ++r) {
            const int gr = arow_base + i * MT + MM::acc_row(lane, r);
            if (gr >= p.M) continue;
            bool zero = false;
            size_t orow = gr;
            if (p.row_len != nullptr) zero = (gr % p.rows_per_item) >= p.row_len[gr / p.rows_per_item];
            if (p.row_map != nullptr) orow = (size_t)p.row_map[gr];
#pragma unroll
            for (int j = 0; j < RN; ++j) {
                const int gc = acol_base + j * MT;
                if (gc < p.N) {
                    float v = act_apply(acc[i][j][r], p.post_act);
                    p.Y[orow * p.ldy + gc] = zero ? 0.f : v;
                }
            }
        }
}

template <int BM, int BN, int WM, int WN, int MT, bool LN>
__global__ __launch_bounds__(WM * WN * 64) void gemm_kernel(const GemmArgs p) { gemm_body<BM, BN, WM, WN, MT, LN>(p); }
template <int BM, int BN, int WM, int WN, int MT, bool LN>
__global__ __launch_bounds__(WM * WN * 64) void gemm_batch_kernel(const GemmBatch b) { gemm_body<BM, BN, WM, WN, MT, LN>(b.a[blockIdx.y]); }

template <int BM, int BN, int WM, int WN, int MT, bool LN>
static int launch_cfg(const GemmArgs& a, hipStream_t stream) {
    const int nbm = (a.M + BM - 1) / BM, nbn = (a.N + BN - 1) / BN;
    hipLaunchKernelGGL((gemm_kernel<BM, BN, WM, WN, MT, LN>), dim3(nbm * nbn), dim3(WM * WN * 64), 0, stream, a);
    LADIFF_LAUNCH_CHECK();
    return 0;
}
template <int BM, int BN, int WM, int WN, int MT, bool LN>
static int launch_cfg_batch(const GemmBatch& b, int n, hipStream_t stream) {
    const int nbm = (b.a[0].M + BM - 1) / BM, nbn = (b.a[0].N + BN - 1) / BN;
    hipLaunchKernelGGL((gemm_batch_kernel<BM, BN, WM, WN, MT, LN>), dim3(nbm * nbn, n), dim3(WM * WN * 64), 0, stream, b);
    LADIFF_LAUNCH_CHECK();
    return 0;
}

int launch_gemm(const GemmArgs& a0, hipStream_t stream) {
    GemmArgs a = a0;
    if (a.A2 == nullptr) a.K1 = a.K;
    LADIFF_CHECK_ARG(a.A && a.W && (a.Y || a.Ys) && a.M >= 0 && a.N > 0 && a.K > 0);
    if (a.M == 0) return 0;
    if (a.split) return gemm_big_supported(a) ? launch_gemm_big(a, stream) : LADIFF_ERR_SHAPE;
    if (a.Y == nullptr || a.Ys != nullptr) return LADIFF_ERR_ARG;
    if (a.K % BK != 0 || a.K1 % BK != 0 || a.K1 > a.K) return LADIFF_ERR_SHAPE;
    if ((a.lda % 4) || (a.ldw % 4) || (a.A2 && (a.lda2 % 4))) return LADIFF_ERR_SHAPE;
    const bool ln = a.ln_g != nullptr;
    if (!ln && (a.ln2_g || a.mod)) return LADIFF_ERR_ARG;
    if (ln && (a.N != 256 || a.ln_b == nullptr)) return LADIFF_ERR_SHAPE;
    if (gemm_big_supported(a)) return launch_gemm_big(a, stream);
    if (ln) {
        if (a.N != 256 || a.ln_b == nullptr) return LADIFF_ERR_SHAPE;
        if (a.M >= 4096) return launch_cfg<64, 256, 2, 1, 32, true>(a, stream);
        return launch_cfg<16, 256, 1, 4, 16, true>(a, stream);
    }
    if (a.M >= 4096) return launch_cfg<128, 128, 2, 2, 32, false>(a, stream);
    if (a.N >= 512) return launch_cfg<64, 64, 2, 2, 32, false>(a, stream);
    return launch_cfg<32, 32, 2, 2, 16, false>(a, stream);
}

int launch_gemm_batch(const GemmArgs* list, int n, hipStream_t stream) {
    LADIFF_CHECK_ARG(list != nullptr && n >= 1 && n <= GEMM_BATCH_MAX);
    GemmBatch b;
    for (int i = 0; i < n; ++i) {
        GemmArgs a = list[i];
        if (a.A2 == nullptr) a.K1 = a.K;
        LADIFF_CHECK_ARG(a.A && a.W && (a.Y || a.Ys) && (a.split || (a.Y && !a.Ys)) && a.M >= 0 && a.N > 0 && a.K > 0);
        LADIFF_CHECK_ARG(a.M == list[0].M && a.N == list[0].N && a.K == list[0].K && (a.ln_g != nullptr) == (list[0].ln_g != nullptr) &&
                         a.split == list[0].split);
        if (a.K % BK != 0 || a.K1 % BK != 0 || a.K1 > a.K) return LADIFF_ERR_SHAPE;
        if ((a.lda % 4) || (a.ldw % 4) || (a.A2 && (a.lda2 % 4))) return LADIFF_ERR_SHAPE;
        if (a.ln_g == nullptr && (a.ln2_g || a.mod)) return LADIFF_ERR_ARG;
        if (a.ln_g != nullptr && (a.N != 256 || a.ln_b == nullptr)) return LADIFF_ERR_SHAPE;
        b.a[i] = a;
    }
    const GemmArgs& a = b.a[0];
    if (a.M == 0) return 0;
    if (a.split) {
        for (int i = 0; i < n; ++i)
            if (!gemm_big_supported(b.a[i])) return LADIFF_ERR_SHAPE;
        return launch_gemm_big_batch(b, n, stream);
    }
    if (gemm_big_supported(a)) return launch_gemm_big_batch(b, n, stream);
    if (a.ln_g != nullptr) {
        if (a.M >= 4096) return launch_cfg_batch<64, 256, 2, 1, 32, true>(b, n, stream);
        return launch_cfg_batch<16, 256, 1, 4, 16, true>(b, n, stream);
    }
    if (a.M >= 4096) return launch_cfg_batch<128, 128, 2, 2, 32, false>(b, n, stream);
    if (a.N >= 512) return launch_cfg_batch<64, 64, 2, 2, 32, false>(b, n, stream);
    return launch_cfg_batch<32, 32, 2, 2, 16, false>(b, n, stream);
}

}
```

### ladiff_amd/csrc/gemm_big.hip

```cpp
#include "gemm.h"

namespace ladiff {

namespace {
constexpr int BKB = 32;
template <int N> __device__ __forceinline__ void wait_vm() { asm volatile("s_waitcnt vmcnt(%0)" ::"n"(N) : "memory"); }
__device__ __forceinline__ void dma16(const float* g, float* l) {
    __builtin_amdgcn_global_load_lds(g, (__attribute__((address_space(3))) void*)l, 16, 0, 0);
}
}

template <int BM, int BN, int WM, int WN, bool LN>
__device__ __forceinline__ void gemm_big_body(const GemmArgs& p) {
    constexpr int NW = 4;
    static_assert(WM * WN == NW, "four waves");
    constexpr int TMW = BM / WM, TNW = BN / WN, RM = TMW / 32, RN = TNW / 32;
    constexpr int ROWS = BM + BN;
    constexpr int STAGE = ROWS * BKB;
    constexpr int GRP = 8 * NW;
    constexpr int GA = BM / GRP, GT = ROWS / GRP;
    static_assert(BM % GRP == 0 && BN % GRP == 0, "tiles are multiples of 32 rows");
    constexpr int CLD = BN + 4;
    constexpr int LDSF = (2 * STAGE > BM * CLD) ? 2 * STAGE : BM * CLD;
    constexpr int LPR = BN / 4;
// ... 53 lines not shown
#pragma unroll
            for (int i = 0; i < RM; ++i) { const int r = i * 32 + frow; fa[i] = ld4(sa + r * BKB + ((c ^ ((r >> 1) & 7)) << 2)); }
#pragma unroll
            for (int j = 0; j < RN; ++j) { const int r = j * 32 + frow; fb[j] = ld4(sb + r * BKB + ((c ^ ((r >> 1) & 7)) << 2)); }
#pragma unroll
            for (int e = 0; e < 4; ++e)
#pragma unroll
                for (int i = 0; i < RM; ++i)
#pragma unroll
                    for (int j = 0; j < RN; ++j)
                        acc[i][j] = __builtin_amdgcn_mfma_f32_32x32x2f32(fa[i][e], fb[j][e], acc[i][j], 0, 0, 0);
        }
    };

    const int er = wave * (BM / NW) + lane / LPR;
    const int ec = 4 * (lane % LPR);
    f32x4 rv[EI];
#pragma unroll
    for (int e = 0; e < EI; ++e) rv[e] = f32x4{0.f, 0.f, 0.f, 0.f};

    issue(0, 0);
    for (int kt = 0; kt < nk; ++kt) {
        const int buf = kt & 1;
        wait_vm<0>();
        __builtin_amdgcn_s_barrier();
        if (kt + 1 < nk) issue(kt + 1, buf ^ 1);
        if (kt == nk - 1 && p.res != nullptr) {
#pragma unroll
            for (int e = 0; e < EI; ++e) {
                const int gr = row0 + er + e * RPI;
                if (gr < p.M) rv[e] = ld4(p.res + (size_t)gr * p.ldres + col0 + ec);
            }
        }
        compute(buf);
    }
    __builtin_amdgcn_s_barrier();

    float* ct = lds;
#pragma unroll
    for (int i = 0; i < RM; ++i)
#pragma unroll
        for (int j = 0; j < RN; ++j)
#pragma unroll
            for (int r = 0; r < 16; ++r)
                ct[(wm * TMW + i * 32 + (r & 3) + 8 * (r >> 2) + 4 * (lane >> 5)) * CLD + wn * TNW + j * 32 + (lane & 31)] = acc[i][j][r];
    asm volatile("s_waitcnt vmcnt(0) lgkmcnt(0)" ::: "memory");
    __builtin_amdgcn_s_barrier();
#pragma unroll
    for (int e = 0; e < EI; ++e) reg_touch(rv[e]);

    f32x4 bv = {0.f, 0.f, 0.f, 0.f};
    if (p.bias != nullptr) bv = ld4(p.bias + col0 + ec);
    f32x4 g1 = bv, b1 = bv, g2 = bv, b2 = bv;
    if constexpr (LN) {
        g1 = ld4(p.ln_g + ec); b1 = ld4(p.ln_b + ec);
        if (p.ln2_g != nullptr) { g2 = ld4(p.ln2_g + ec); b2 = ld4(p.ln2_b + ec); }
    }
    act_dispatch(p.act, [&](auto ACT) __attribute__((always_inline)) {
#pragma unroll
    for (int e = 0; e < EI; ++e) {
        const int lr = er + e * RPI;
        const int gr = row0 + lr;
        f32x4 v = ld4(ct + lr * CLD + ec);
#pragma unroll
        for (int q = 0; q < 4; ++q) v[q] = act_c<decltype(ACT)::value>(v[q] + bv[q]) + rv[e][q];
        if constexpr (LN) {
#pragma unroll
            for (int pass = 0; pass < 2; ++pass) {
                if (pass == 1 && p.ln2_g == nullptr) break;
                const float mean = wave_sum((v[0] + v[1]) + (v[2] + v[3])) * (1.f / 256.f);
                float sq = 0.f;
#pragma unroll
                for (int q = 0; q < 4; ++q) { const float d = v[q] - mean; sq += d * d; }
                const float rstd = rsqrtf(wave_sum(sq) * (1.f / 256.f) + LN_EPS);
#pragma unroll
                for (int q = 0; q < 4; ++q) v[q] = (v[q] - mean) * rstd * (pass ? g2[q] : g1[q]) + (pass ? b2[q] : b1[q]);
            }
        }
        if (gr < p.M) st4(p.Y + (size_t)gr * p.ldy + col0 + ec, v);
    }
    });
}

template <int BM, int BN>
__device__ __forceinline__ void gemm_big_split_body(const GemmArgs& p) {
    constexpr int NW = 4, WM = 2, WN = 2;
    constexpr int TMW = BM / WM, TNW = BN / WN, RM = TMW / 16, RN = TNW / 16;
    constexpr int ROWS = BM + BN;
    constexpr int STAGE = ROWS * 32;
    constexpr int GRP = 8 * NW;
    constexpr int GA = BM / GRP, GT = ROWS / GRP;
    constexpr int CLD = BN + 4;
    constexpr int LPR = BN / 4, RPI = 64 / LPR, EI = BM / NW / RPI;
    constexpr int LDSF = (2 * STAGE > BM * CLD) ? 2 * STAGE : BM * CLD;

    __shared__ __attribute__((aligned(1024))) float lds[LDSF];

    const int tid = threadIdx.x, lane = tid & 63;
    const int wave = __builtin_amdgcn_readfirstlane(tid >> 6);
    const int wm = wave / WN, wn = wave % WN;
    const int argM = pin_s(p.M), argK1 = pin_s(p.K1), ldy = pin_s(p.ldy), act = pin_s(p.act);
    float* const argY = pin_s(p.Y); float* const argYs = pin_s(p.Ys);
    const int nbn = p.N / BN;
    const int nbm = (argM + BM - 1) / BM;
    const int xcd = blockIdx.x & 7, local = blockIdx.x >> 3;
    const int bm = (local / nbn) * 8 + xcd, bn = local % nbn;
    if (bm >= nbm) return;
    const int row0 = bm * BM, col0 = bn * BN;
    const int ksplit = pin_s(p.ksplit), kz = ksplit > 1 ? (int)blockIdx.y : 0;
    const int nk_all = p.K / 32, nk = nk_all / ksplit, kt0 = kz * nk;

    const int rl = 8 * wave + (lane >> 3);
    const int cs = (lane & 7) ^ ((rl >> 1) & 7);
    const int kl = (cs < 4 ? cs * 4 : 32 + (cs - 4) * 4);
    float* const lbase = lds + 8 * wave * 32;
    auto issue = [&](int ktl, int buf) __attribute__((always_inline)) {
        const int kt = kt0 + ktl;
        const int k0 = (kt >> 1) * 64, hf = (kt & 1) * 16;
        const float* abase; int ald;
        if (k0 < argK1) { abase = p.A + k0; ald = p.lda; } else { abase = p.A2 + (k0 - argK1); ald = p.lda2; }
#pragma unroll
        for (int g = 0; g < GT; ++g) {
            const float* src;
            if (g < GA) {
                int gr = row0 + GRP * g + rl; gr = gr < argM ? gr : argM - 1;
                src = abase + (size_t)gr * ald + hf + kl;
            } else {
                src = p.W + (size_t)(col0 + GRP * (g - GA) + rl) * p.ldw + k0 + hf + kl;
            }
            dma16(src, lbase + buf * STAGE + GRP * g * 32);
        }
    };

    f32x4 acc[RM][RN];
#pragma unroll
    for (int i = 0; i < RM; ++i)
#pragma unroll
        for (int j = 0; j < RN; ++j) acc[i][j] = f32x4{0.f, 0.f, 0.f, 0.f};

    const int frow = lane & 15, fk = lane >> 4;
    const int sw = (frow >> 1) & 7;
    auto compute = [&](int buf) __attribute__((always_inline)) {
        const float* sa = lds + buf * STAGE + (wm * TMW) * 32;
        const float* sb = lds + buf * STAGE + (BM + wn * TNW) * 32;
        s16x8 ah[RM], al[RM], bh[RN], bl[RN];
#pragma unroll
        for (int i = 0; i < RM; ++i) {
            const int r = i * 16 + frow;
            ah[i] = __builtin_bit_cast(s16x8, ld4(sa + r * 32 + ((fk ^ sw) << 2)));
            al[i] = __builtin_bit_cast(s16x8, ld4(sa + r * 32 + (((4 + fk) ^ sw) << 2)));
        }
#pragma unroll
        for (int j = 0; j < RN; ++j) {
            const int r = j * 16 + frow;
            bh[j] = __builtin_bit_cast(s16x8, ld4(sb + r * 32 + ((fk ^ sw) << 2)));
            bl[j] = __builtin_bit_cast(s16x8, ld4(sb + r * 32 + (((4 + fk) ^ sw) << 2)));
        }
#pragma unroll
        for (int i = 0; i < RM; ++i)
#pragma unroll
            for (int j = 0; j < RN; ++j) acc[i][j] = MFMA16_S16(al[i], bh[j], acc[i][j], 0, 0, 0);
#pragma unroll
        for (int i = 0; i < RM; ++i)
#pragma unroll
            for (int j = 0; j < RN; ++j) acc[i][j] = MFMA16_S16(ah[i], bl[j], acc[i][j], 0, 0, 0);
#pragma unroll
        for (int i = 0; i < RM; ++i)
#pragma unroll
            for (int j = 0; j < RN; ++j) acc[i][j] = MFMA16_S16(ah[i], bh[j], acc[i][j], 0, 0, 0);
    };

    const int er = wave * (BM / NW) + lane / LPR;
    const int ec = 4 * (lane % LPR);
    f32x4 rv[EI];
#pragma unroll
    for (int e = 0; e < EI; ++e) rv[e] = f32x4{0.f, 0.f, 0.f, 0.f};
    f32x4 bv = {0.f, 0.f, 0.f, 0.f};

    issue(0, 0);
    for (int kt = 0; kt < nk; ++kt) {
        const int buf = kt & 1;
        wait_vm<0>();
        __builtin_amdgcn_s_barrier();
        if (kt + 1 < nk) issue(kt + 1, buf ^ 1);
        if (kt == nk - 1 && ksplit == 1) {
            if (p.bias != nullptr) bv = ld4(p.bias + col0 + ec);
            if (p.res != nullptr) {
#pragma unroll
                for (int e = 0; e < EI; ++e) {
                    const int gr = row0 + er + e * RPI;
                    if (gr < argM) rv[e] = ld4(p.res + (size_t)gr * p.ldres + col0 + ec);
                }
            }
        }
        compute(buf);
    }
    __builtin_amdgcn_s_barrier();

    float* ct = lds;
#pragma unroll
    for (int i = 0; i < RM; ++i)
#pragma unroll
        for (int j = 0; j < RN; ++j)
#pragma unroll
            for (int r = 0; r < 4; ++r)
                ct[(wm * TMW + i * 16 + 4 * (lane >> 4) + r) * CLD + wn * TNW + j * 16 + (lane & 15)] = acc[i][j][r];
    asm volatile("s_waitcnt vmcnt(0) lgkmcnt(0)" ::: "memory");
    __builtin_amdgcn_s_barrier();
    reg_touch(bv);
#pragma unroll
    for (int e = 0; e < EI; ++e) reg_touch(rv[e]);

    if (ksplit > 1) {
        float* const Yz = argY + (size_t)kz * p.plane;
#pragma unroll
        for (int e = 0; e < EI; ++e) {
            const int lr = er + e * RPI;
            const int gr = row0 + lr;
            if (gr < argM) st4g(Yz + (size_t)gr * ldy + col0 + ec, ld4(ct + lr * CLD + ec));
        }
        return;
    }
    act_dispatch(act, [&](auto ACT) __attribute__((always_inline)) {
#pragma unroll
        for (int e = 0; e < EI; ++e) {
            const int lr = er + e * RPI;
            const int gr = row0 + lr;
            f32x4 v = ld4(ct + lr * CLD + ec);
#pragma unroll
            for (int q = 0; q < 4; ++q) v[q] = act_c<decltype(ACT)::value>(v[q] + bv[q]) + rv[e][q];
            if (gr < argM) {
                if (argY != nullptr) st4g(argY + (size_t)gr * ldy + col0 + ec, v);
                if (argYs != nullptr) store_split4g(argYs + (size_t)gr * ldy, col0 + ec, v);
            }
        }
    });
}

template <int BM, int BN>
__global__ __launch_bounds__(256, 2) void gemm_big_split_kernel(const GemmArgs p) { gemm_big_split_body<BM, BN>(p); }
template <int BM, int BN>
__global__ __launch_bounds__(256, 2) void gemm_big_split_batch_kernel(const GemmBatch b) { gemm_big_split_body<BM, BN>(b.a[blockIdx.y]); }

template <int BM, int BN, int WM, int WN, bool LN>
__global__ __launch_bounds__(256) void gemm_big_kernel(const GemmArgs p) { gemm_big_body<BM, BN, WM, WN, LN>(p); }
template <int BM, int BN, int WM, int WN, bool LN>
__global__ __launch_bounds__(256) void gemm_big_batch_kernel(const GemmBatch b) { gemm_big_body<BM, BN, WM, WN, LN>(b.a[blockIdx.y]); }

template <int BM, int BN, int WM, int WN, bool LN>
static int launch_big_batch(const GemmBatch& b, int n, hipStream_t s) {
    const GemmArgs& a = b.a[0];
    const int nbm = (a.M + BM - 1) / BM, nbn = a.N / BN;
    const int grid = ((nbm + 7) / 8) * 8 * nbn;
    hipLaunchKernelGGL((gemm_big_batch_kernel<BM, BN, WM, WN, LN>), dim3(grid, n), dim3(256), 0, s, b);
    LADIFF_LAUNCH_CHECK();
    return 0;
}

template <int BM, int BN, int WM, int WN, bool LN>
static int launch_big(const GemmArgs& a, hipStream_t s) {
    const int nbm = (a.M + BM - 1) / BM, nbn = a.N / BN;
    const int grid = ((nbm + 7) / 8) * 8 * nbn;
    hipLaunchKernelGGL((gemm_big_kernel<BM, BN, WM, WN, LN>), dim3(grid), dim3(256), 0, s, a);
    LADIFF_LAUNCH_CHECK();
    return 0;
}

bool gemm_big_supported(const GemmArgs& a) {
    if (a.split) return a.M > 0 && a.K % 64 == 0 && a.K1 % 64 == 0 && a.N % 128 == 0 && a.lda % 4 == 0 && a.ldw % 4 == 0 && (!a.A2 || a.lda2 % 4 == 0) &&
                        a.ldy % 64 == 0 && !a.ln_g && !a.mod && !a.row_len && !a.row_map && a.post_act == ACT_NONE && (a.Y || a.Ys);
    if (a.M < 4096 || a.K % BKB || a.K1 % BKB || (a.lda % 4) || (a.ldw % 4) || (a.A2 && (a.lda2 % 4))) return false;
    if ((a.ldy % 4) || (a.res && (a.ldres % 4)) || a.mod || a.row_len || a.row_map || a.post_act != ACT_NONE) return false;
    if (a.ln_g != nullptr) return a.N == 256;
    return a.N % 128 == 0;
}

int launch_gemm_big(const GemmArgs& a, hipStream_t s) {
    if (a.split) {
        const int nbm = (a.M + 127) / 128, nbn = a.N / 128;
        const int ks = a.ksplit > 1 ? a.ksplit : 1;
        if (ks > 1 && ((a.K / 32) % ks != 0 || a.Y == nullptr || a.Ys != nullptr || a.plane == 0)) return LADIFF_ERR_ARG;
        if (nbm * nbn <= 256 && a.M > 64) {
            const int nbm64 = (a.M + 63) / 64;
            hipLaunchKernelGGL((gemm_big_split_kernel<64, 128>), dim3(((nbm64 + 7) / 8) * 8 * nbn, ks), dim3(256), 0, s, a);
        } else {
            hipLaunchKernelGGL((gemm_big_split_kernel<128, 128>), dim3(((nbm + 7) / 8) * 8 * nbn, ks), dim3(256), 0, s, a);
        }
        LADIFF_LAUNCH_CHECK();
        return 0;
    }
    if (a.ksplit > 1) return LADIFF_ERR_ARG;
    if (a.ln_g != nullptr) return launch_big<64, 256, 2, 2, true>(a, s);
    return launch_big<128, 128, 2, 2, false>(a, s);
}

int launch_gemm_big_batch(const GemmBatch& b, int n, hipStream_t s) {
    for (int i = 0; i < n; ++i) if (b.a[i].ksplit > 1) return LADIFF_ERR_ARG;
    if (b.a[0].split) {
        const GemmArgs& a = b.a[0];
        const int nbm = (a.M + 127) / 128, nbn = a.N / 128;
        hipLaunchKernelGGL((gemm_big_split_batch_kernel<128, 128>), dim3(((nbm + 7) / 8) * 8 * nbn, n), dim3(256), 0, s, b);
        LADIFF_LAUNCH_CHECK();
        return 0;
    }
    if (b.a[0].ln_g != nullptr) return launch_big_batch<64, 256, 2, 2, true>(b, n, s);
    return launch_big_batch<128, 128, 2, 2, false>(b, n, s);
}

}
```

### ladiff_amd/csrc/graph_key.h

```cpp
#pragma once
#include <algorithm>
#include <cstddef>
#include <cstdint>
#include <cstdlib>
#include <cstring>

namespace ladiff {

struct GraphKey {
    static constexpr int CAPACITY = 40;
    uint64_t v[CAPACITY] = {0};
    int n = 0;

    GraphKey& add(uint64_t x) {
        if (n == CAPACITY) std::abort();
        v[n++] = x;
        return *this;
    }
    GraphKey& add(const void* p) { return add((uint64_t) reinterpret_cast<uintptr_t>(p)); }
    GraphKey& add(int x) { return add((uint64_t)(int64_t)x); }
    GraphKey& add(unsigned x) { return add((uint64_t)x); }
    GraphKey& add(float x) {
        uint32_t u;
        static_assert(sizeof(u) == sizeof(x), "float is 32 bits");
// ... 13 lines not shown
}
inline uint64_t weights_hash(const float* const* w, const float* const* w_split, int n) {
    const uint64_t h = fnv1a_ptrs(w, n, 1469598103934665603ull);
    return w_split != nullptr ? fnv1a_ptrs(w_split, n, h ^ 0x9e3779b97f4a7c15ull) : h;
}

struct ReverseArgs {
    const float* const* w;
    const float* const* w_split;
    uint64_t weights_generation;
    const float *text_emb, *init_noise;
    const int32_t *counts, *final_counts, *h_counts;
    const float *sinusoid, *coef, *step_noise;
    float guidance_scale, init_noise_sigma;
    int cfg, B, T, n_text, n_steps;
    float* z;
    void* ws;
    size_t ws_bytes;
    int reuse_time_tables;
    void* stream;
    const float* guidance_scales;
    const uint64_t* seeds;
    const uint32_t* prompt_index;
    int draw_init_noise;
    float* x0_prev;
    const float* z0 = nullptr;
    const int32_t* starts = nullptr;
    int first_step = 0;
    float* traj_x = nullptr;
    float* traj_x0 = nullptr;
};

inline GraphKey sampler_key(const ReverseArgs& a, int n_params, bool pipeline, int plan_mr, int plan_nb, const unsigned noise[4]) {
    GraphKey k;
    k.add(a.ws);
    k.add(a.counts);
    k.add(a.final_counts);
    k.add(a.coef);
    k.add(a.step_noise);
    k.add(a.stream);
    k.add(a.text_emb);
    k.add(a.init_noise);
    k.add(a.z);
    k.add(a.B);
    k.add(a.T);
    k.add(a.n_steps);
    k.add(a.cfg);
    k.add(a.n_text);
    k.add(a.w_split != nullptr ? 1 : 0);
    k.add(pipeline ? 1 : 0);
    k.add(pipeline ? plan_mr : 0);
    k.add(pipeline ? plan_nb : 0);
    k.add(a.guidance_scale);
    k.add(a.init_noise_sigma);
    for (int i = 0; i < 4; ++i) k.add(pipeline ? 0u : noise[i]);
    k.add(weights_hash(a.w, a.w_split, n_params));
    k.add(a.weights_generation);
    k.add(a.guidance_scales);
    k.add(a.seeds);
    k.add(a.prompt_index);
    k.add(a.draw_init_noise);
    if (a.x0_prev != nullptr) k.add(a.x0_prev);
    if (a.z0 != nullptr) {
        k.add(a.z0);
        k.add(a.starts);
        k.add(!pipeline || a.starts == nullptr ? a.first_step : -1);
    }
    if (a.traj_x != nullptr || a.traj_x0 != nullptr) {
        k.add((uint64_t)0x7472616a);
        k.add(a.traj_x);
        k.add(a.traj_x0);
    }
    return k;
}

struct DecSwitches {
    int fused_mlp;
    int small_rows_path;
    int final_split;
    int out_cross;
    int fused_attn;
    int mlp_variant;
    int post_off;
};
constexpr int DEC_SMALL_ROWS = 4096;
struct DecRoute { bool small, fused_attn, out_cross, fused_mlp, final_split, post; };
inline DecRoute dec_route(bool split_mode, int rows, const DecSwitches& sw, int mlp_min_rows) {
    DecRoute r;
    r.small = split_mode && rows < DEC_SMALL_ROWS && sw.small_rows_path;
    r.fused_attn = split_mode && sw.fused_attn && (rows >= DEC_SMALL_ROWS || sw.fused_attn == 2);
    r.out_cross = split_mode && !r.small && sw.out_cross;
    r.fused_mlp = split_mode && sw.fused_mlp && (rows >= mlp_min_rows || sw.fused_mlp == 2);
    r.final_split = split_mode && rows >= DEC_SMALL_ROWS && sw.final_split;
    r.post = r.out_cross && r.fused_mlp && !r.small && !sw.post_off;
    return r;
}
inline GraphKey decode_key(const float* const* w, const float* const* w_split, int n_params, uint64_t weights_generation, const float* z,
                           const int32_t* lengths, const int32_t* counts, const int32_t* row_off, int total_rows, int B, int F, int T, int C,
                           const float* feats, const void* ws, const void* stream, const DecSwitches& sw) {
    GraphKey k;
    k.add(z);
    k.add(lengths);
    k.add(counts);
    k.add(row_off);
    k.add(feats);
    k.add(ws);
    k.add(stream);
    k.add(B);
    k.add(F);
    k.add(T);
    k.add(C);
    k.add(total_rows);
    k.add(w_split != nullptr ? 1 : 0);
    k.add(sw.fused_mlp);
    k.add(sw.small_rows_path);
    k.add(sw.final_split);
    k.add(sw.mlp_variant);
    k.add(sw.fused_attn);
    k.add(sw.out_cross);
    k.add(sw.post_off);
    k.add(weights_hash(w, w_split, n_params));
    k.add(weights_generation);
    return k;
}

}
```

### ladiff_amd/csrc/kernels.h

```cpp
#pragma once
#include "common.h"
#include "noise_gen.h"

namespace ladiff {

enum RedMode : int { RED_PLAIN = 0, RED_LN = 1, RED_LN_ADD = 2, RED_LN_MOD = 3 };
struct RedArgs {
    const float* P = nullptr;
    const float* bias = nullptr; const float* res = nullptr;
    const float* g = nullptr; const float* b = nullptr;
    const float* tab = nullptr;
    const int32_t* d_step = nullptr;
    const int32_t* counts = nullptr;
    float* out = nullptr; float* outs = nullptr;
    const int32_t* d_base = nullptr;
    const float* g2 = nullptr; const float* b2 = nullptr;
    size_t plane = 0;
    int S = 1, mode = RED_PLAIN, tab_step_stride = 0, Bs = 1, T = 1, pad_row = 0, b_off = 0, M = 0;
};
int launch_reduce_rows(const RedArgs& a, hipStream_t s, bool per_sample = false);
int launch_split_rows(const float* x, float* y, int R, int K, hipStream_t s);
int launch_gather_rows(const float* src, const int32_t* index, int n_rows, int row_floats, float* dst, hipStream_t s);
int launch_split_range_stats(const float* const* xs, const int64_t* counts, int n, int64_t max_count, unsigned long long* stats,
                             hipStream_t s);
int launch_layernorm(const float* x, const float* g, const float* b, float* y, int M, hipStream_t s);
constexpr int DEC_PREP_MAX = 9;
struct DecCrossPrepBatch { const float* kv[DEC_PREP_MAX]; const float* wq[DEC_PREP_MAX]; const float* bq[DEC_PREP_MAX];
                           const float* wo[DEC_PREP_MAX]; float* gu[DEC_PREP_MAX]; };
constexpr int ROW_BATCH_MAX = 9;
struct RowBatch { const float* a[ROW_BATCH_MAX]; const float* g[ROW_BATCH_MAX]; const float* b[ROW_BATCH_MAX]; float* y[ROW_BATCH_MAX]; };
int launch_layernorm_batch(const RowBatch& rb, int n, int M, hipStream_t s);
int launch_ca_table_input_batch(const RowBatch& rb, int n_layers, int step_stride, int n, int B2, hipStream_t s, int split_out = 0);
int launch_ca_table_input(const float* nval, const float* beta, const float* mod, int step_stride, int n, int B2, float* u,
                          hipStream_t s);
int launch_add_pe(const float* sample, const float* pe, int Bs, int b_off, int b_n, int T, float* x, float* xs, hipStream_t s);
int launch_broadcast_pe(const float* pe, int B, int F, float* x, float* xs, hipStream_t s);
int launch_broadcast_pe_ragged(const float* pe, const int32_t* row_off, int B, int F, int F_out, float* x, float* xs, int32_t* row_out,
                               hipStream_t s);
int launch_relu(const float* x, float* y, size_t n, hipStream_t s);
int launch_pad_rows(const float* src, const float* srcb, float* dst, float* dstb, int C, int Np, hipStream_t s);
int launch_zero_fill(float* x, size_t n, hipStream_t s);
int launch_silu(const float* x, float* y, size_t n, hipStream_t s);
int launch_sinusoid(const int64_t* t, int n, float* out, hipStream_t s);
struct StepEnd {
    const float *coef, *noise;
    NoiseGen gen;
    float g; const float* gs;
    int cfg;
    float* x0_prev;
    bool edit; const int32_t* starts; int first_step;
    float *traj_x, *traj_x0; const int32_t* traj_counts;
    bool record() const { return traj_x != nullptr || traj_x0 != nullptr; }
};
int launch_traj_zero_pad(float* traj, const int32_t* counts, int first, int n, int B, int T, hipStream_t s);
int launch_cfg_step(const float* eps, float* lat, const int32_t* d_step, const StepEnd& e, int B, int T, hipStream_t s);
int launch_advance(int32_t* d_step, hipStream_t s);
int launch_step_tail(float* x, float* xs, const float* ng, const float* nb, float* lat, int32_t* d_step, const float* pe, const StepEnd& e,
                     int B, int T, hipStream_t s);
int launch_noise_fill(const NoiseGen& gen, int step0, int n, int B, int T, float* out, hipStream_t s);
int launch_init_latents(const float* noise, const int32_t* counts, float sigma, float* lat, int B, int T, hipStream_t s);
int launch_init_latents_gen(const NoiseGen& gen, const int32_t* counts, float sigma, float* lat, int B, int T, hipStream_t s);
int launch_init_latents_from(const float* z0, const float* noise, const NoiseGen& gen, const int32_t* counts, const float* coef,
                             const int32_t* starts, int first_step, float* lat, int B, int T, int32_t* d_step, hipStream_t s);
int launch_finalize_latents(const float* lat, const int32_t* counts, float* z, int B, int T, hipStream_t s, const unsigned* status = nullptr);

int launch_dec_qkv_attn(const float* xs, const float* w, const float* bias, const int32_t* lengths, const int32_t* row_off, float* out,
                        int B, int F, int split_out, hipStream_t s);
int launch_scatter_feats(const float* tmp, int ldt, int C, int M, int F, const int32_t* row_len, const int32_t* row_map, float* feats,
                         hipStream_t s);
int launch_pad_cols(const float* x, float* y, int R, int C, int Cp, hipStream_t s);
int launch_dvae_pad_cols(const float* x, const int32_t* slot, const float* values, int n, float* y, int B, int F, int C, int Cp,
                         hipStream_t s);
int launch_encoder_assemble(const float* token, const float* emb, const float* pe, const int32_t* lengths,
                            const int32_t* counts, int B, int F, int T, float* x, float* xs, uint32_t* keybits, hipStream_t s);
int launch_encoder_finalize(const float* out, const float* eps, const int32_t* counts, int B, int T, int S, float* mu, float* sd,
                            float* latent, hipStream_t s);

int launch_lca_kv(const float* key, const float* value, int B, int N, float* att, hipStream_t s);
int launch_lca_apply(const float* q, const float* att, const int32_t* counts, int Bs, int b_off, int b_n, int T, const float* mod,
                     int step_stride, int sample_stride, const int32_t* d_step, const float* g, const float* be, float* u,
                     hipStream_t s);
int launch_denoiser_self_attention_general(const float* qkv, const float* text_kv, int N, const float* tables, int kv_off,
                                           int step_stride, const int32_t* d_step, const int32_t* counts, int Bs, int b_off,
                                           int b_n, int T, float* out, hipStream_t s);

int launch_decoder_cross_prep(const DecCrossPrepBatch& pb, int n, int B, int T, hipStream_t s);
int launch_decoder_out_cross(const float* att_s, const float* x0, const float* wo_s, const float* bo, const float* g1, const float* b1,
                             const float* bo_c, const float* g2, const float* b2, const int32_t* counts, int B, int F, int T,
                             const float* gu_ws, float* y, float* ys, hipStream_t s, const int32_t* row_off);
int launch_decoder_cross_apply(const float* x, const float* bo, const float* g2, const float* b2, const int32_t* counts, int B, int F,
                               int T, const float* gu_ws, float* y, float* ys, hipStream_t s, const int32_t* row_off = nullptr,
                               const float* g1 = nullptr, const float* b1 = nullptr);
int launch_decoder_cross_maps(const float* x, const int32_t* counts, const int32_t* lengths, int B, int F, int T, const float* gu_ws,
                              float* maps, hipStream_t s, const int32_t* row_off, const float* g1, const float* b1);

int launch_feats2joints(const float* feats, const float* mean, const float* stdv, int B, int F, int C, int J, float* joints,
                        hipStream_t s);

int launch_joints2feats(const float* joints, const int32_t* h_lengths, int B, int L, const float* tgt, float feet_thre, const float* mean,
                        const float* stdv, float* feats, hipStream_t s);

int launch_joint_ape_ave(const float* rst, const float* ref, const int32_t* lengths, int B, int F, int J, const int32_t* part_idx,
                         float factor, float* seq_rows, double* acc, hipStream_t s);
int launch_joint_mr(const float* rst, const float* ref, int B, int F, int J, float* seq_rows, double* acc, hipStream_t s);

int launch_vae_losses(const float* m_rst, const float* m_ref, size_t n_feat, const float* j_rst, const float* j_ref, size_t n_joint,
                      const float* mu, const float* sd, size_t n_lat, double l_rec, double l_joint, double l_kl, double* part, int blocks,
                      double* batch, double* acc, hipStream_t s);

int launch_denoiser_self_attention(const float* qkv, const float* text_kv, const float* tables, int kv_off,
                                   int step_stride, const int32_t* d_step, const int32_t* counts, int Bs, int b_off,
                                   int b_n, int T, float* out, int split_out, hipStream_t s);
int launch_decoder_self_attention(const float* qkv, const int32_t* lengths, const uint32_t* keybits, float* out, int B, int F,
                                  int split_out, hipStream_t s, const int32_t* row_off = nullptr, int shared_qkv = 0);
int launch_self_attention(const float* qkv, const int32_t* lengths, const uint32_t* keybits, float* out, int B, int F, int nheads,
                          int causal, int split_out, hipStream_t s, const int32_t* row_off = nullptr);
int launch_self_attention_split(const float* qkv, const int32_t* lengths, const uint32_t* keybits, float* out, int B, int F,
                                 int nheads, int causal, int split_out, hipStream_t s, const int32_t* row_off = nullptr, int shared_qkv = 0);
int launch_decoder_cross_attention(const float* q, const float* kv, const int32_t* counts, float* out, int B, int F,
                                   int T, int split_out, hipStream_t s);

}
```

### ladiff_amd/csrc/model.h

```cpp
#pragma once
#include <atomic>
#include "graph_key.h"
#include "seq.h"
#include "systolic_plan.h"
#include "workspace.h"

namespace ladiff {

int denoiser_time_tables(const DenoiserW& w, const float* sinus, int n, float* tables, float* ws, size_t ws_floats, hipStream_t s);
int denoiser_text_cache(const DenoiserW& w, const float* text, int B2, const float* tables, int n_steps, float* cache,
                        float* ws, size_t ws_floats, hipStream_t s, int ntxt = 1);
int denoiser_forward(const DenoiserW& w, const DenoiserW* w_split, const float* tables, const int32_t* d_step,
                     const float* cache, int n_steps, const float* sample, int Bs, int dup, int T, const int32_t* counts, float* eps, float* ws,
                     size_t ws_floats, hipStream_t s, int b_lo = 0, int b_n = -1, int loop_mode = 0, int ntxt = 1,
                     const int32_t* d_base = nullptr, const float* dctab = nullptr);
int denoiser_text_static(const DenoiserW& w, const float* text, int B2, float* cache, float* ws, size_t ws_floats, hipStream_t s);
int denoiser_ctab(const DenoiserW& w, const float* tables_lo, int n, float* cache, int B2, float* u, size_t u_floats, hipStream_t s,
                  const DenoiserW* w_split = nullptr);
int linear_cross_attention(const DenoiserW& w, int layer, const float* x, const float* xf, const float* emb, const int32_t* counts,
                           int B, int T, int N, float* out, float* ws, size_t ws_floats, hipStream_t s);

int denoiser_forward_timesteps(const DenoiserW& w, const DenoiserW* w_split, const float* text, const int64_t* timesteps, const float* sample,
                               int B2, int T, const int32_t* counts, float* eps, float* ws, size_t ws_floats, hipStream_t s);
int launch_q_sample(const float* z, const int64_t* ts, const float* acp, int n_train, const int32_t* counts, const NoiseGen& gen, float* noise,
                    float* noisy, int B, int T, hipStream_t s);
int launch_diffusion_losses(const float* pred, const float* noise, size_t n, double lambda_inst, double* part, int blocks, double* batch,
                            double* acc, hipStream_t s);

struct Sampler;
int diffusion_reverse(Sampler* sp, const DenoiserW& w, const DenoiserW* w_split, const ReverseArgs& a);

struct DecSwitchAtoms {
    std::atomic<int> fused_mlp{1}, small_rows_path{1}, final_split{1}, out_cross{1}, fused_attn{1}, mlp_variant{0}, post_off{0};
    DecSwitches snapshot() const { return {fused_mlp, small_rows_path, final_split, out_cross, fused_attn, mlp_variant, post_off}; }
};
extern DecSwitchAtoms g_dec;
int dec_mlp_prepare();
int dec_qkv_attn_prepare();
int dec_cross_prepare();
int dec_mlp_min_rows();
int vae_decode(const DecoderW& w, const DecoderW* w_split, const float* z, const int32_t* lengths, const int32_t* counts,
               const int32_t* row_off, int R, int B, int F, int T, int C, float* feats, float* ws, size_t ws_floats, hipStream_t s, const DecSwitches& sw,
               float* att_maps = nullptr);

int launch_dec_mlp(const float* xs, const float* x, const float* w1, const float* b1, const float* w2, const float* b2, const float* g3,
                   const float* be3, const float* g4, const float* be4, float* y, float* ys, int M, hipStream_t s, int variant);

struct DecPostArgs {
    const float* att;
    const float* x0;
    const float* wo;
    const float *bo, *g1, *be1;
    const float *gu, *cc;
    const float *bo_c, *g2, *be2;
    const int32_t *counts, *row_off;
    const float *w1, *b1, *w2, *b2, *g3, *be3, *g4, *be4;
    float *y, *ys;
    int B, F, T, M;
};
int dec_post_prepare();
int launch_dec_post_gu(float* guws, size_t gu_layer, int n, int B, int T, hipStream_t s);
int launch_dec_post(const DecPostArgs& a, hipStream_t s);

int vae_encode(const EncoderW& w, const EncoderW* w_split, const float* features, const int32_t* lengths,
               const int32_t* counts, const float* eps, int B, int F, int T, int C, float* mu, float* sd, float* latent, float* ws,
               size_t ws_floats, hipStream_t s, const int32_t* slot = nullptr, const float* values = nullptr, int n_values = 0);

#ifdef LADIFF_STAMPS
extern unsigned long long* g_sys_stamps;
extern int g_sys_probe;
#endif
bool sys_supported(int B, int T, int cfg, bool split);
int sys_reset_status(float* ws, hipStream_t s);
int sys_build_stages(const DenoiserW& W, const DenoiserW& WS, float* ws, int MR, int NB, std::vector<unsigned char>& host);
int launch_systolic_loop(const DenoiserW& W, float* ws, const float* tables, const float* tkv, const float* ctab, int n_ctab, float* lat,
                         const int32_t* counts, const StepEnd& e, int B, int T, int step_lo, int n, int fp32, int MR, int NB, hipStream_t s,
                         int fault_wg, unsigned long long timeout_ticks);

int launch_qkv_attention(const float* x, const float* w, const float* bias, const float* text_kv, const float* tables,
                         int kv_off, int step_stride, const int32_t* d_step, const int32_t* counts, int Bs, int b_off,
                         int b_n, int T, float* out, hipStream_t s);

int clip_text_encode(const ClipW& w, const ClipW* w_split, int n_layers, int vocab, const int64_t* ids, int B, int S, int L,
                     float* out, float* ws, size_t ws_floats, hipStream_t s, const int32_t* seq_len = nullptr,
                     const int32_t* row_off = nullptr, const int32_t* row_seq = nullptr, int total_rows = 0);

const std::vector<std::string>& t2m_move_param_names();
const std::vector<std::string>& t2m_motion_param_names();
const std::vector<std::string>& t2m_text_param_names();
int t2m_movement_encode(const float* const* w, const float* feats, int ld, int B, int F, int Cin, float* out, float* ws,
                        size_t ws_floats, hipStream_t s);
int t2m_motion_encode(const float* const* w, const float* mov, const int32_t* m_lens, int B, int T, float* out, float* ws,
                      size_t ws_floats, hipStream_t s);
int t2m_text_encode(const float* const* w, const float* word_embs, const float* pos_onehot, const int32_t* cap_lens, int B, int L,
                    float* out, float* ws, size_t ws_floats, hipStream_t s);

}
```

### ladiff_amd/csrc/rowops.hip

```cpp
#include <algorithm>

#include "kernels.h"
#include "step_rule.h"

namespace ladiff {

constexpr int ROWS_PER_BLOCK = 4;

__device__ __forceinline__ void row_stats(const f32x4 v, float& mean, float& rstd) {
    float s = wave_sum(v[0] + v[1] + v[2] + v[3]);
    mean = s * (1.f / 256.f);
    float q = 0.f;
#pragma unroll
    for (int i = 0; i < 4; ++i) { const float d = v[i] - mean; q += d * d; }
    q = wave_sum(q);
    rstd = rsqrtf(q * (1.f / 256.f) + LN_EPS);
}

__global__ __launch_bounds__(256) void layernorm_kernel(const float* __restrict__ x, const float* __restrict__ g,
                                                        const float* __restrict__ b, float* __restrict__ y, int M) {
    const int row = blockIdx.x * ROWS_PER_BLOCK + (threadIdx.x >> 6);
    const int c = (threadIdx.x & 63) * 4;
    if (row >= M) return;
    f32x4 v = ld4(x + (size_t)row * D + c);
// ... 36 lines not shown
template <bool PER_SAMPLE>
__global__ __launch_bounds__(256) void reduce_rows_kernel(const RedArgs p) {
    const float* const P = pin_s(p.P); const float* const bias = pin_s(p.bias); const float* const res = pin_s(p.res);
    const float* const g = pin_s(p.g); const float* const b = pin_s(p.b); const float* const tab = pin_s(p.tab);
    const int32_t* const d_step = pin_s(p.d_step); const int32_t* const counts = pin_s(p.counts);
    const int32_t* const d_base = pin_s(p.d_base);
    float* const out = pin_s(p.out); float* const outs = pin_s(p.outs);
    const size_t plane = pin_s(p.plane);
    const int S = pin_s(p.S), mode = pin_s(p.mode), tab_step_stride = pin_s(p.tab_step_stride), Bs = pin_s(p.Bs),
              T = pin_s(p.T), pad_row = pin_s(p.pad_row), b_off = pin_s(p.b_off), M = pin_s(p.M);
    const int row = blockIdx.x * ROWS_PER_BLOCK + (threadIdx.x >> 6);
    const int c = (threadIdx.x & 63) * 4;
    if (row >= M) return;
    const f32x4 zero = {0.f, 0.f, 0.f, 0.f};
    const float* prow = P + (size_t)row * D + c;
    f32x4 pl[4];
#pragma unroll
    for (int s = 0; s < 4; ++s) pl[s] = s < S ? ld4g(prow + s * plane) : zero;
    const f32x4 bi = bias != nullptr ? ld4g(bias + c) : zero;
    const f32x4 rs = res != nullptr ? ld4g(res + (size_t)row * D + c) : zero;
    f32x4 gg = zero, bb = zero, gg2 = zero, bb2 = zero;
    if (mode != RED_PLAIN) { gg = ld4g(g + c); bb = ld4g(b + c); }
    const bool twice = mode == RED_LN && p.g2 != nullptr;
    if (twice) { gg2 = ld4g(p.g2 + c); bb2 = ld4g(p.b2 + c); }
    int step = d_step != nullptr ? *(const __attribute__((address_space(1))) int32_t*)d_step : 0;
    if (d_base != nullptr) step -= *(const __attribute__((address_space(1))) int32_t*)d_base;
    const int b2 = b_off + row / T, tt = row % T;
    if (PER_SAMPLE) step = b2;
    int cnt = 0x7fffffff;
    if (mode == RED_LN_ADD && counts != nullptr) cnt = *(const __attribute__((address_space(1))) int32_t*)(counts + b2 % Bs);
    const float* t = tab + (size_t)step * tab_step_stride;
    f32x4 t0 = zero, t1 = zero;
    if (mode == RED_LN_ADD) { t0 = ld4g(t + (size_t)(PER_SAMPLE ? 0 : b2) * D + c); t1 = ld4g(t + (size_t)pad_row * D + c); }
    else if (mode == RED_LN_MOD) { t0 = ld4g(t + c); t1 = ld4g(t + 256 + c); }

    f32x4 v;
#pragma unroll
    for (int i = 0; i < 4; ++i) v[i] = ((pl[0][i] + pl[1][i]) + pl[2][i]) + pl[3][i] + bi[i] + rs[i];
    if (mode != RED_PLAIN) {
        float mean, rstd;
        row_stats(v, mean, rstd);
#pragma unroll
        for (int i = 0; i < 4; ++i) v[i] = (v[i] - mean) * rstd * gg[i] + bb[i];
        if (twice) {
            row_stats(v, mean, rstd);
#pragma unroll
            for (int i = 0; i < 4; ++i) v[i] = (v[i] - mean) * rstd * gg2[i] + bb2[i];
        }
        if (mode == RED_LN_ADD) {
            const bool valid = tt < cnt;
#pragma unroll
            for (int i = 0; i < 4; ++i) v[i] += valid ? t0[i] : t1[i];
        } else if (mode == RED_LN_MOD) {
#pragma unroll
            for (int i = 0; i < 4; ++i) v[i] = silu(v[i] * (1.f + t0[i]) + t1[i]);
        }
    }
    if (out != nullptr) st4g(out + (size_t)row * D + c, v);
    if (outs != nullptr) store_split4g(outs + (size_t)row * D, c, v);
}

int launch_reduce_rows(const RedArgs& args, hipStream_t s, bool per_sample) {
    if (args.S < 1 || args.S > 4) return LADIFF_ERR_SHAPE;
    RedArgs a = args;
    a.plane = (size_t)a.M * D;
    const dim3 grid((a.M + ROWS_PER_BLOCK - 1) / ROWS_PER_BLOCK), block(256);
    if (per_sample) hipLaunchKernelGGL(reduce_rows_kernel<true>, grid, block, 0, s, a);
    else hipLaunchKernelGGL(reduce_rows_kernel<false>, grid, block, 0, s, a);
    LADIFF_LAUNCH_CHECK();
    return 0;
}

__global__ __launch_bounds__(256) void ca_table_input_kernel(const float* __restrict__ nval, const float* __restrict__ beta,
                                                             const float* __restrict__ mod, int step_stride, int B2, int M,
                                                             float* __restrict__ u) {
    const int row = blockIdx.x * ROWS_PER_BLOCK + (threadIdx.x >> 6);
    const int c = (threadIdx.x & 63) * 4;
    if (row >= M) return;
    const int step = row / (B2 + 1), b = row % (B2 + 1);
    const float* m = mod + (size_t)step * step_stride;
    const f32x4 sc = ld4(m + c), sh = ld4(m + 256 + c);
    f32x4 v = b < B2 ? ld4(nval + (size_t)b * D + c) : ld4(beta + c);
#pragma unroll
    for (int i = 0; i < 4; ++i) v[i] = silu(v[i] * (1.f + sc[i]) + sh[i]);
    st4(u + (size_t)row * D + c, v);
}
__global__ __launch_bounds__(256) void ca_table_input_batch_kernel(const RowBatch rb, int step_stride, int B2, int M, int split_out) {
    const int row = blockIdx.x * ROWS_PER_BLOCK + (threadIdx.x >> 6);
    const int c = (threadIdx.x & 63) * 4;
    if (row >= M) return;
    const int k = blockIdx.y;
    const int step = row / (B2 + 1), b = row % (B2 + 1);
    const float* m = rb.b[k] + (size_t)step * step_stride;
    const f32x4 sc = ld4(m + c), sh = ld4(m + 256 + c);
    f32x4 v = b < B2 ? ld4(rb.a[k] + (size_t)b * D + c) : ld4(rb.g[k] + c);
#pragma unroll
    for (int i = 0; i < 4; ++i) v[i] = silu(v[i] * (1.f + sc[i]) + sh[i]);
    if (split_out) store_split4(rb.y[k] + (size_t)row * D, c, v);
    else st4(rb.y[k] + (size_t)row * D + c, v);
}
int launch_ca_table_input_batch(const RowBatch& rb, int n_layers, int step_stride, int n, int B2, hipStream_t s, int split_out) {
    const int M = n * (B2 + 1);
    if (M == 0 || n_layers == 0) return 0;
    LADIFF_CHECK_ARG(n_layers >= 1 && n_layers <= ROW_BATCH_MAX);
    hipLaunchKernelGGL(ca_table_input_batch_kernel, dim3((M + ROWS_PER_BLOCK - 1) / ROWS_PER_BLOCK, n_layers), dim3(256), 0, s, rb,
                       step_stride, B2, M, split_out);
    LADIFF_LAUNCH_CHECK();
    return 0;
}

int launch_ca_table_input(const float* nval, const float* beta, const float* mod, int step_stride, int n, int B2, float* u,
                          hipStream_t s) {
    const int M = n * (B2 + 1);
    hipLaunchKernelGGL(ca_table_input_kernel, dim3((M + ROWS_PER_BLOCK - 1) / ROWS_PER_BLOCK), dim3(256), 0, s, nval, beta, mod,
                       step_stride, B2, M, u);
    LADIFF_LAUNCH_CHECK();
    return 0;
}

__global__ __launch_bounds__(256) void add_pe_kernel(const float* __restrict__ sample, const float* __restrict__ pe,
                                                     int Bs, int T, int M, int b_off, float* __restrict__ x, float* __restrict__ xs) {
    const int row = blockIdx.x * ROWS_PER_BLOCK + (threadIdx.x >> 6);
    const int c = (threadIdx.x & 63) * 4;
    if (row >= M) return;
    const int b2 = b_off + row / T, t = row % T;
    f32x4 v = ld4(sample + ((size_t)(b2 % Bs) * T + t) * D + c);
    const f32x4 p = ld4(pe + (size_t)t * D + c);
#pragma unroll
    for (int i = 0; i < 4; ++i) v[i] += p[i];
    st4(x + (size_t)row * D + c, v);
    if (xs != nullptr) store_split4(xs + (size_t)row * D, c, v);
}

int launch_add_pe(const float* sample, const float* pe, int Bs, int b_off, int b_n, int T, float* x, float* xs, hipStream_t s) {
    const int M = b_n * T;
    hipLaunchKernelGGL(add_pe_kernel, dim3((M + ROWS_PER_BLOCK - 1) / ROWS_PER_BLOCK), dim3(256), 0, s, sample, pe, Bs, T, M, b_off, x, xs);
    LADIFF_LAUNCH_CHECK();
    return 0;
}

__global__ __launch_bounds__(256) void broadcast_pe_kernel(const float* __restrict__ pe, int F, int M, float* __restrict__ x,
                                                           float* __restrict__ xs) {
    const int row = blockIdx.x * ROWS_PER_BLOCK + (threadIdx.x >> 6);
    const int c = (threadIdx.x & 63) * 4;
    if (row >= M) return;
    const f32x4 v = ld4(pe + (size_t)(row % F) * D + c);
    st4(x + (size_t)row * D + c, v);
    if (xs != nullptr) store_split4(xs + (size_t)row * D, c, v);
}

__global__ __launch_bounds__(256) void broadcast_pe_ragged_kernel(const float* __restrict__ pe, const int32_t* __restrict__ row_off,
                                                                  int F, int F_out, float* __restrict__ x, float* __restrict__ xs,
                                                                  int32_t* __restrict__ row_out) {
    const int b = blockIdx.y, f = blockIdx.x * ROWS_PER_BLOCK + (threadIdx.x >> 6);
    const int c = (threadIdx.x & 63) * 4;
    const int r0 = row_off[b];
    if (f >= F || f >= row_off[b + 1] - r0) return;
    const size_t row = (size_t)r0 + f;
    const f32x4 v = ld4(pe + (size_t)f * D + c);
    st4(x + row * D + c, v);
    if (xs != nullptr) store_split4(xs + row * D, c, v);
    if (c == 0) row_out[row] = b * F_out + f;
}
int launch_broadcast_pe_ragged(const float* pe, const int32_t* row_off, int B, int F, int F_out, float* x, float* xs, int32_t* row_out,
                               hipStream_t s) {
    if (B == 0) return 0;
    hipLaunchKernelGGL(broadcast_pe_ragged_kernel, dim3((F + ROWS_PER_BLOCK - 1) / ROWS_PER_BLOCK, B), dim3(256), 0, s, pe, row_off, F,
                       F_out, x, xs, row_out);
    LADIFF_LAUNCH_CHECK();
    return 0;
}

int launch_broadcast_pe(const float* pe, int B, int F, float* x, float* xs, hipStream_t s) {
    const int M = B * F;
    hipLaunchKernelGGL(broadcast_pe_kernel, dim3((M + ROWS_PER_BLOCK - 1) / ROWS_PER_BLOCK), dim3(256), 0, s, pe, F, M, x, xs);
    LADIFF_LAUNCH_CHECK();
    return 0;
}

__global__ __launch_bounds__(256) void gather_rows_kernel(const float* __restrict__ src, const int32_t* __restrict__ index, int n_rows,
                                                          int row4, float* __restrict__ dst) {
    const int row = blockIdx.x * ROWS_PER_BLOCK + (threadIdx.x >> 6);
    if (row >= n_rows) return;
    const float* s = src + (size_t)index[row] * row4 * 4;
    float* d = dst + (size_t)row * row4 * 4;
    for (int c = threadIdx.x & 63; c < row4; c += 64) st4(d + c * 4, ld4(s + c * 4));
}
int launch_gather_rows(const float* src, const int32_t* index, int n_rows, int row_floats, float* dst, hipStream_t s) {
    if (n_rows == 0) return 0;
    hipLaunchKernelGGL(gather_rows_kernel, dim3((n_rows + ROWS_PER_BLOCK - 1) / ROWS_PER_BLOCK), dim3(256), 0, s, src, index, n_rows,
                       row_floats / 4, dst);
    LADIFF_LAUNCH_CHECK();
    return 0;
}

__global__ __launch_bounds__(256) void split_rows_kernel(const float* __restrict__ x, float* __restrict__ y, int K, size_t n4) {
    const size_t i = (size_t)blockIdx.x * 256 + threadIdx.x;
    if (i >= n4) return;
    const size_t row = (i * 4) / K;
    const int k = (int)((i * 4) % K);
    store_split4(y + row * K, k, ld4(x + i * 4));
}
int launch_split_rows(const float* x, float* y, int R, int K, hipStream_t s) {
    const size_t n4 = (size_t)R * K / 4;
    hipLaunchKernelGGL(split_rows_kernel, dim3((unsigned)((n4 + 255) / 256)), dim3(256), 0, s, x, y, K, n4);
    LADIFF_LAUNCH_CHECK();
    return 0;
}

#ifndef LADIFF_SPLIT_BF16
constexpr float SPLIT_EXACT_MAX = 65504.f;
#else
constexpr float SPLIT_EXACT_MAX = 3.402823466e38f;
#endif

struct SplitRangeAcc {
    float max_abs = 0.f, max_err = 0.f;
    uint32_t nonfinite = 0, beyond = 0, coarse = 0;
    __device__ __forceinline__ void add(float x, float hi, float lo) {
        const float ax = fabsf(x);
        if (!(ax <= 3.402823466e38f)) {
            ++nonfinite;
            if (ax == __builtin_huge_valf()) max_abs = ax;
            return;
        }
        max_abs = fmaxf(max_abs, ax);
        if (ax > SPLIT_EXACT_MAX) ++beyond;
        const float err = fabsf((x - hi) - lo);
        max_err = fmaxf(max_err, err);
        if (ax != 0.f && err > ax * 0x1p-11f) ++coarse;
    }
};

__global__ __launch_bounds__(256) void split_range_stats_kernel(const float* const* __restrict__ xs, const int64_t* __restrict__ counts,
                                                                unsigned long long* __restrict__ stats) {
    const int t = blockIdx.y;
    const int64_t c = counts[t];
    if (c <= 0) return;
    const float* __restrict__ x = xs[t];
    const size_t n = (size_t)c, stride = (size_t)gridDim.x * 256;
    const size_t tid = (size_t)blockIdx.x * 256 + threadIdx.x;
    const size_t n4 = (reinterpret_cast<uintptr_t>(x) & 15) == 0 ? n / 4 : 0;
    SplitRangeAcc a;
    for (size_t i = tid; i < n4; i += stride) {
        const f32x4 v = ld4(x + i * 4);
        s16x4 hi, lo;
        split4(v, hi, lo);
#pragma unroll
        for (int j = 0; j < 4; ++j) a.add(v[j], (float)hi[j], (float)lo[j]);
    }
    for (size_t i = n4 * 4 + tid; i < n; i += stride) {
        const float v = x[i];
        s16x2 hi, lo;
        split2(v, 0.f, hi, lo);
        a.add(v, (float)hi[0], (float)lo[0]);
    }
    const float m = wave_max_nonneg(a.max_abs), e = wave_max_nonneg(a.max_err);
    const uint32_t nf = wave_sum_u32(a.nonfinite), nb = wave_sum_u32(a.beyond), nc = wave_sum_u32(a.coarse);
// ... 488 lines not shown
```

Measured before the change: 11150 motions/s.

## Generate operands in-kernel: dedupe layer-0 decoder attention, fuse ctab input, direct final store

Three changes remove memory round-trips. In decoder layer 0 the query input is identical for items with equal length, so a leader kernel maps each item to a representative; self-attention runs only for leaders and the post kernel reads the leader's attention rows. The denoiser cross-attn table input (silu of modulated values) is now computed inside the split GEMM's A-load instead of being written by a separate kernel. The final decoder projection stores directly into output features with row mapping instead of going through a scatter pass. A debug mask can restore the old memory-operand paths. The cost is more complex GEMM kernels, and the dedup depends on layer-0 inputs truly matching across items.

New measurement: 11190 motions/s, median of 6. Within noise of the previous version (+0.3%).

```diff
diff --git a/include/ladiff_hip_debug.h b/include/ladiff_hip_debug.h
--- a/include/ladiff_hip_debug.h
+++ b/include/ladiff_hip_debug.h
@@ -16,6 +16,7 @@
 LADIFF_API int ladiff_debug_set_xcd_local(int on);
 LADIFF_API int ladiff_debug_set_decoder_fusion(int on);
 LADIFF_API int ladiff_debug_set_mlp_variant(int v);
+LADIFF_API int ladiff_debug_set_memory_operands(int mask);
 
 LADIFF_API int ladiff_debug_set_loop_thresholds(int look_ahead_from, int small_upto);
 LADIFF_API int ladiff_debug_set_graph_epoch_rule(int on);
diff --git a/ladiff_amd/_lib.py b/ladiff_amd/_lib.py
--- a/ladiff_amd/_lib.py
+++ b/ladiff_amd/_lib.py
@@ -175,6 +175,7 @@
     "ladiff_debug_set_xcd_local": (c_int, [c_int]),
     "ladiff_debug_set_decoder_fusion": (c_int, [c_int]),
     "ladiff_debug_set_mlp_variant": (c_int, [c_int]),
+    "ladiff_debug_set_memory_operands": (c_int, [c_int]),
     "ladiff_reverse_plan": (c_int, [c_int, c_int, c_void_p, c_int, c_int, c_int, c_int, c_void_p, c_void_p]),
     "ladiff_decoder_graph_create": (c_int, [ctypes.POINTER(c_void_p)]),
     "ladiff_decoder_graph_destroy": (c_int, [c_void_p]),
diff --git a/ladiff_amd/csrc/api.hip b/ladiff_amd/csrc/api.hip
--- a/ladiff_amd/csrc/api.hip
+++ b/ladiff_amd/csrc/api.hip
@@ -312,6 +312,13 @@
     g_dec.small_rows_path = (on & 4) ? 0 : 1;
     g_dec.final_split = (on & 8) ? 0 : 1;
     g_dec.fused_attn = (on & 16) ? 0 : (on & 32) ? 2 : 1;
+    return 0;
+}
+
+int ladiff_debug_set_memory_operands(int mask) {
+    LADIFF_CHECK_ARG(mask >= 0 && (mask & ~(1 | DEC_MEM_LAYER0 | DEC_MEM_FINAL)) == 0);
+    g_ctab_through_memory = mask & 1;
+    g_dec.memory_operands = mask & (DEC_MEM_LAYER0 | DEC_MEM_FINAL);
     return 0;
 }
 
diff --git a/ladiff_amd/csrc/attention.hip b/ladiff_amd/csrc/attention.hip
--- a/ladiff_amd/csrc/attention.hip
+++ b/ladiff_amd/csrc/attention.hip
@@ -152,7 +152,8 @@
 __global__ __launch_bounds__(NT, NT == 64 ? 2 : 1) void self_attn_split_kernel(const float* __restrict__ qkv, const int32_t* __restrict__ lengths,
                                                                const uint32_t* __restrict__ keybits, float* __restrict__ out,
                                                                int B, int F, int split_out, const AttnGeom g,
-                                                               const int32_t* __restrict__ row_off, int shared_qkv) {
+                                                               const int32_t* __restrict__ row_off, int shared_qkv,
+                                                               const int32_t* __restrict__ leader) {
     constexpr int NKT = FM / 32, IT = FM * 16 / NT, VLD = FM + 8;
     static_assert(FM % 32 == 0 && (FM * 16) % NT == 0 && NT % 64 == 0 && (FM / 4) % (NT / 64) == 0 && NT / 64 >= FM / 32, "a wave per query tile");
     __shared__ __attribute__((aligned(16))) s16 Kp[2 * FM * DH];
@@ -162,6 +163,7 @@
     float* const Vtmp = reinterpret_cast<float*>(Kp);
     const int tid = threadIdx.x, lane = tid & 63, wave = tid >> 6;
     const int b = blockIdx.x / g.nheads, h = blockIdx.x % g.nheads;
+    if (leader != nullptr && leader[b] != b) return;
     int len = F;
     uint32_t kb[NKT + 1];
     if (keybits != nullptr) {
@@ -347,13 +349,14 @@
 }
 
 int launch_self_attention_split(const float* qkv, const int32_t* lengths, const uint32_t* keybits, float* out, int B, int F,
-                                 int nheads, int causal, int split_out, hipStream_t s, const int32_t* row_off, int shared_qkv) {
+                                 int nheads, int causal, int split_out, hipStream_t s, const int32_t* row_off, int shared_qkv,
+                                 const int32_t* leader) {
     if (F > SA_FMAX || F < 1 || nheads < 1) return LADIFF_ERR_SHAPE;
     if (B == 0) return 0;
     const int W = nheads * DH;
     const AttnGeom g{nheads, 3 * W, W, 2 * W, W, causal};
-    if (F <= 32) hipLaunchKernelGGL((self_attn_split_kernel<32, 64>), dim3(B * nheads), dim3(64), 0, s, qkv, lengths, keybits, out, B, F, split_out, g, row_off, shared_qkv);
-    else hipLaunchKernelGGL((self_attn_split_kernel<SA_FMAX, 512>), dim3(B * nheads), dim3(512), 0, s, qkv, lengths, keybits, out, B, F, split_out, g, row_off, shared_qkv);
+    if (F <= 32) hipLaunchKernelGGL((self_attn_split_kernel<32, 64>), dim3(B * nheads), dim3(64), 0, s, qkv, lengths, keybits, out, B, F, split_out, g, row_off, shared_qkv, leader);
+    else hipLaunchKernelGGL((self_attn_split_kernel<SA_FMAX, 512>), dim3(B * nheads), dim3(512), 0, s, qkv, lengths, keybits, out, B, F, split_out, g, row_off, shared_qkv, leader);
     LADIFF_LAUNCH_CHECK();
     return 0;
 }
diff --git a/ladiff_amd/csrc/common.h b/ladiff_amd/csrc/common.h
--- a/ladiff_amd/csrc/common.h
+++ b/ladiff_amd/csrc/common.h
@@ -85,6 +85,7 @@
 }
 
 __device__ __forceinline__ float silu(float v) { return v / (1.f + expf(-v)); }
+__device__ __forceinline__ float ca_table_value(float nv, float scale, float shift) { return silu(nv * (1.f + scale) + shift); }
 
 template <int WIDTH>
 __device__ __forceinline__ float group_sum(float v) {
diff --git a/ladiff_amd/csrc/dec_post.hip b/ladiff_amd/csrc/dec_post.hip
--- a/ladiff_amd/csrc/dec_post.hip
+++ b/ladiff_amd/csrc/dec_post.hip
@@ -89,10 +89,17 @@
     nrows = tile_ok ? nrows : 0;
     const int row0 = srow + f0;
     const int myrow = nrows > 0 ? row0 + (frow < nrows ? frow : nrows - 1) : M - 1;
+    int arow = myrow, xrow = myrow;
+    if (p.leader != nullptr) {
+        const int lb = p.leader[b];
+        const int lrow = p.row_off != nullptr ? p.row_off[lb] : lb * p.F;
+        xrow = nrows > 0 ? myrow - srow : 0;
+        arow = __builtin_amdgcn_readfirstlane(nrows > 0 ? lrow : 0) + xrow;
+    }
 
     s16x8 xh[8], xl[8];
     {
-        const char* xr = reinterpret_cast<const char*>(p.att) + (size_t)myrow * 1024 + fk * 16;
+        const char* xr = reinterpret_cast<const char*>(p.att) + (size_t)arow * 1024 + fk * 16;
 #pragma unroll
         for (int s = 0; s < 8; ++s) {
             xh[s] = *reinterpret_cast<const s16x8*>(xr + (s >> 1) * 256 + (s & 1) * 64);
@@ -101,7 +108,7 @@
     }
     f32x4 hacc[8], oacc[16];
 #pragma unroll
-    for (int jj = 0; jj < 16; ++jj) oacc[jj] = ld4(p.x0 + (size_t)myrow * D + 32 * (jj >> 1) + 8 * fk + 4 * (jj & 1));
+    for (int jj = 0; jj < 16; ++jj) oacc[jj] = ld4(p.x0 + (size_t)xrow * D + 32 * (jj >> 1) + 8 * fk + 4 * (jj & 1));
     float cv[8];
     {
         const float* cb = p.cc + (size_t)b * (H * T) + fk * T;
diff --git a/ladiff_amd/csrc/decoder.hip b/ladiff_amd/csrc/decoder.hip
--- a/ladiff_amd/csrc/decoder.hip
+++ b/ladiff_amd/csrc/decoder.hip
@@ -32,6 +32,8 @@
     DecSwitches swr = sw;
     if (att_maps != nullptr) swr.out_cross = 0;
     const DecRoute rt = dec_route(sp, M, swr, dec_mlp_min_rows());
+    const bool l0s = rt.layer0_shared && (size_t)B <= (size_t)M * D;
+    int32_t* const leader = l0s ? reinterpret_cast<int32_t*>(a.P[0]) : nullptr;
     const Seq c{sp, M, s};
     const DecoderW& wm = mfma_table(w, wsp);
     Twin P[4], SK[NSKIP];
@@ -79,7 +81,7 @@
             return 0;
         } else if (rt.small) { LADIFF_TRY(krs(cur, D, in, q, 3 * D, 3 * D, ACT_NONE, nullptr, M)); DEC_CUT(); }
         else { LADIFF_TRY(launch_gemm(proj(c, cur, D, in, q, 3 * D, 3 * D), s)); DEC_CUT(); }
-        if (sp) { LADIFF_TRY(launch_self_attention_split(q.f, lengths, nullptr, att, B, F, H, 0, 1, s, row_off, shared)); DEC_CUT(); }
+        if (sp) { LADIFF_TRY(launch_self_attention_split(q.f, lengths, nullptr, att, B, F, H, 0, 1, s, row_off, shared, shared ? leader : nullptr)); DEC_CUT(); }
         else { LADIFF_TRY(launch_decoder_self_attention(q.f, lengths, nullptr, att, B, F, 0, s, row_off, shared)); DEC_CUT(); }
         return 0;
     };
@@ -126,14 +128,16 @@
     auto post_attention = [&](Twin dst) -> int {
         const LinearW out = out_proj(L.self_attn); const float* gu = guws + l * a.gu_layer;
         const NormW* fin = l == NL - 1 ? &w.norm : nullptr;
-        const DecPostArgs pa{att, cur.f, out.w, out.b, L.norm1.g, L.norm1.b, gu, gu + (size_t)B * H * T * 2 * D, L.cross_attn.out_b, L.norm2.g,
+        const bool l0 = l == 0 && l0s;
+        const DecPostArgs pa{att, l0 ? pex.f : cur.f, out.w, out.b, L.norm1.g, L.norm1.b, gu, gu + (size_t)B * H * T * 2 * D, L.cross_attn.out_b, L.norm2.g,
                              L.norm2.b, counts, row_off, L.lin1.w, L.lin1.b, L.lin2.w, L.lin2.b, L.norm3.g, L.norm3.b,
-                             fin ? fin->g : nullptr, fin ? fin->b : nullptr, dst.f, dst.s, B, F, T, M};
+                             fin ? fin->g : nullptr, fin ? fin->b : nullptr, dst.f, dst.s, B, F, T, M, l0 ? leader : nullptr};
         LADIFF_TRY(launch_dec_post(pa, s)); DEC_CUT();
         return 0;
     };
 
-    if (ragged) { LADIFF_TRY(launch_broadcast_pe_ragged(w.query_pe, row_off, B, F, F, P[0].f, P[0].s, a.row_out, s)); DEC_CUT(); }
+    if (l0s) { LADIFF_TRY(launch_dec_leader(lengths, row_off, B, F, F, leader, ragged ? a.row_out : nullptr, s)); DEC_CUT(); }
+    else if (ragged) { LADIFF_TRY(launch_broadcast_pe_ragged(w.query_pe, row_off, B, F, F, P[0].f, P[0].s, a.row_out, s)); DEC_CUT(); }
     else { LADIFF_TRY(launch_broadcast_pe(w.query_pe, B, F, P[0].f, P[0].s, s)); DEC_CUT(); }
     for (l = 0; l < NL; ++l) {
         L = mixed(w.layer[l], wm.layer[l]);
@@ -152,6 +156,13 @@
         if ((size_t)M * Np > a.hid_floats || (size_t)Np * (D + 1) > a.qkv_floats) return LADIFF_ERR_SHAPE;
         float* wpad = qkv; float* bpad = qkv + (size_t)Np * D;
         LADIFF_TRY(launch_pad_rows(wm.final_layer.w, w.final_layer.b, wpad, bpad, C, Np, s)); DEC_CUT();
+        if (rt.final_direct) {
+            GemmArgs g = proj(c, cur, D, LinearW{wpad, bpad}, Twin{feats, nullptr}, C, Np);
+            g.direct_cols = C;
+            if (ragged) g.row_map = a.row_out;
+            else { g.row_len = lengths; g.rows_per_item = F; }
+            return launch_gemm(g, s);
+        }
         LADIFF_TRY(launch_gemm(proj(c, cur, D, LinearW{wpad, bpad}, Twin{hid, nullptr}, Np, Np), s)); DEC_CUT();
         return launch_scatter_feats(hid, Np, C, M, F, ragged ? nullptr : lengths, ragged ? a.row_out : nullptr, feats, s);
     }
diff --git a/ladiff_amd/csrc/denoiser.hip b/ladiff_amd/csrc/denoiser.hip
--- a/ladiff_amd/csrc/denoiser.hip
+++ b/ladiff_amd/csrc/denoiser.hip
@@ -133,6 +133,7 @@
     return launch_gemm_batch(val, NL, s);
 }
 
+std::atomic<int> g_ctab_through_memory{0};
 int denoiser_ctab(const DenoiserW& w, const float* tables_lo, int n, float* cache, int B2, float* u, size_t u_floats, hipStream_t s,
                   const DenoiserW* wsp) {
     const int R = B2 + 1;
@@ -144,6 +145,7 @@
     if (u_floats >= u_all) {
         RowBatch rb;
         GemmArgs g[NL];
+        const bool in_kernel = wsp != nullptr && !g_ctab_through_memory;
         for (int l = 0; l < NL; ++l) {
             const DenLayerW& L = w.layer[l];
             float* ul = u + (size_t)l * n * R * D;
@@ -151,8 +153,9 @@
             rb.b[l] = tables_lo + (size_t)l * DEN_LAYER_STRIDE + DEN_OFF_CA_MOD; rb.y[l] = ul;
             g[l] = lin(ul, D, L.ca_proj.out, ctab + (size_t)l * n * R * D, D, n * R, D, D);
             if (wsp != nullptr) { g[l].W = wsp->layer[l].ca_proj.out.w; g[l].split = 1; }
-        }
-        LADIFF_TRY(launch_ca_table_input_batch(rb, NL, DEN_STEP_STRIDE, n, B2, s, wsp != nullptr ? 1 : 0));
+            if (in_kernel) { g[l].gen_nval = rb.a[l]; g[l].gen_beta = rb.g[l]; g[l].gen_mod = rb.b[l]; g[l].gen_stride = DEN_STEP_STRIDE; g[l].gen_B2 = B2; }
+        }
+        if (!in_kernel) LADIFF_TRY(launch_ca_table_input_batch(rb, NL, DEN_STEP_STRIDE, n, B2, s, wsp != nullptr ? 1 : 0));
         return launch_gemm_batch(g, NL, s);
     }
     for (int l = 0; l < NL; ++l) {
diff --git a/ladiff_amd/csrc/gemm.h b/ladiff_amd/csrc/gemm.h
--- a/ladiff_amd/csrc/gemm.h
+++ b/ladiff_amd/csrc/gemm.h
@@ -23,6 +23,9 @@
     const int32_t* row_len = nullptr; int rows_per_item = 0;
     const int32_t* row_map = nullptr;
     int ksplit = 1; size_t plane = 0;
+    int direct_cols = 0;
+    const float* gen_nval = nullptr; const float* gen_beta = nullptr; const float* gen_mod = nullptr;
+    int gen_stride = 0, gen_B2 = 0;
 };
 
 int launch_gemm(const GemmArgs& a, hipStream_t stream);
diff --git a/ladiff_amd/csrc/gemm.hip b/ladiff_amd/csrc/gemm.hip
--- a/ladiff_amd/csrc/gemm.hip
+++ b/ladiff_amd/csrc/gemm.hip
@@ -286,7 +286,7 @@
     LADIFF_CHECK_ARG(a.A && a.W && (a.Y || a.Ys) && a.M >= 0 && a.N > 0 && a.K > 0);
     if (a.M == 0) return 0;
     if (a.split) return gemm_big_supported(a) ? launch_gemm_big(a, stream) : LADIFF_ERR_SHAPE;
-    if (a.Y == nullptr || a.Ys != nullptr) return LADIFF_ERR_ARG;
+    if (a.Y == nullptr || a.Ys != nullptr || a.direct_cols > 0 || a.gen_nval != nullptr) return LADIFF_ERR_ARG;
     if (a.K % BK != 0 || a.K1 % BK != 0 || a.K1 > a.K) return LADIFF_ERR_SHAPE;
     if ((a.lda % 4) || (a.ldw % 4) || (a.A2 && (a.lda2 % 4))) return LADIFF_ERR_SHAPE;
     const bool ln = a.ln_g != nullptr;
@@ -325,6 +325,7 @@
             if (!gemm_big_supported(b.a[i])) return LADIFF_ERR_SHAPE;
         return launch_gemm_big_batch(b, n, stream);
     }
+    if (a.gen_nval != nullptr) return LADIFF_ERR_ARG;
     if (gemm_big_supported(a)) return launch_gemm_big_batch(b, n, stream);
     if (a.ln_g != nullptr) {
         if (a.M >= 4096) return launch_cfg_batch<64, 256, 2, 1, 32, true>(b, n, stream);
diff --git a/ladiff_amd/csrc/gemm_big.hip b/ladiff_amd/csrc/gemm_big.hip
--- a/ladiff_amd/csrc/gemm_big.hip
+++ b/ladiff_amd/csrc/gemm_big.hip
@@ -159,7 +159,7 @@
     });
 }
 
-template <int BM, int BN>
+template <int BM, int BN, bool DIRECT = false, bool AGEN = false>
 __device__ __forceinline__ void gemm_big_split_body(const GemmArgs& p) {
     constexpr int NW = 4, WM = 2, WN = 2;
     constexpr int TMW = BM / WM, TNW = BN / WN, RM = TMW / 16, RN = TNW / 16;
@@ -197,7 +197,7 @@
         const float* abase; int ald;
         if (k0 < argK1) { abase = p.A + k0; ald = p.lda; } else { abase = p.A2 + (k0 - argK1); ald = p.lda2; }
 #pragma unroll
-        for (int g = 0; g < GT; ++g) {
+        for (int g = AGEN ? GA : 0; g < GT; ++g) {
             const float* src;
             if (g < GA) {
                 int gr = row0 + GRP * g + rl; gr = gr < argM ? gr : argM - 1;
@@ -209,6 +209,44 @@
         }
     };
 
+    constexpr int GI = BM * 4 / 256;
+    const float* gsrc[GI]; const float* gmod[GI]; int goff[GI];
+    if constexpr (AGEN) {
+        const int R = p.gen_B2 + 1;
+#pragma unroll
+        for (int it = 0; it < GI; ++it) {
+            const int item = tid + 256 * it, r = item >> 2, g = item & 3;
+            int gr = row0 + r; gr = gr < argM ? gr : argM - 1;
+            const int step = gr / R, b = gr - step * R;
+            gsrc[it] = (b < p.gen_B2 ? p.gen_nval + (size_t)b * 256 : p.gen_beta) + 8 * g;
+            gmod[it] = p.gen_mod + (size_t)step * p.gen_stride + 8 * g;
+            goff[it] = r * 32 + ((g ^ ((r >> 1) & 7)) << 2);
+        }
+    }
+    auto gen_a = [&](int ktl, int buf) __attribute__((always_inline)) {
+        const int kc = (ktl >> 1) * 64 + (ktl & 1) * 32;
+        f32x4 v[GI][6];
+#pragma unroll
+        for (int it = 0; it < GI; ++it) {
+            v[it][0] = ld4(gsrc[it] + kc); v[it][1] = ld4(gsrc[it] + kc + 4);
+            v[it][2] = ld4(gmod[it] + kc); v[it][3] = ld4(gmod[it] + kc + 4);
+            v[it][4] = ld4(gmod[it] + 256 + kc); v[it][5] = ld4(gmod[it] + 256 + kc + 4);
+        }
+#pragma unroll
+        for (int it = 0; it < GI; ++it) {
+#pragma unroll
+            for (int e = 0; e < 4; ++e) {
+                v[it][0][e] = ca_table_value(v[it][0][e], v[it][2][e], v[it][4][e]);
+                v[it][1][e] = ca_table_value(v[it][1][e], v[it][3][e], v[it][5][e]);
+            }
+            s16x8 hi, lo;
+            split8(v[it][0], v[it][1], hi, lo);
+            float* dst = lds + buf * STAGE + goff[it];
+            *reinterpret_cast<s16x8*>(dst) = hi;
+            *reinterpret_cast<s16x8*>(lds + buf * STAGE + (goff[it] ^ 16)) = lo;
+        }
+    };
+
     f32x4 acc[RM][RN];
 #pragma unroll
     for (int i = 0; i < RM; ++i)
@@ -253,14 +291,39 @@
 #pragma unroll
     for (int e = 0; e < EI; ++e) rv[e] = f32x4{0.f, 0.f, 0.f, 0.f};
     f32x4 bv = {0.f, 0.f, 0.f, 0.f};
-
+    int drow = -1, dval = 0;
+    float bd[BN / 64];
+#pragma unroll
+    for (int h = 0; h < BN / 64; ++h) bd[h] = 0.f;
+
+    if constexpr (AGEN) {
+        wait_vm<0>();
+        gen_a(0, 0);
+        __builtin_amdgcn_sched_barrier(0);
+    }
     issue(0, 0);
     for (int kt = 0; kt < nk; ++kt) {
         const int buf = kt & 1;
-        wait_vm<0>();
+        if constexpr (AGEN) asm volatile("s_waitcnt vmcnt(0) lgkmcnt(0)" ::: "memory");
+        else wait_vm<0>();
         __builtin_amdgcn_s_barrier();
+        if constexpr (AGEN) {
+            if (kt + 1 < nk) { gen_a(kt + 1, buf ^ 1); __builtin_amdgcn_sched_barrier(0); }
+        }
         if (kt + 1 < nk) issue(kt + 1, buf ^ 1);
-        if (kt == nk - 1 && ksplit == 1) {
+        if constexpr (DIRECT) {
+            if (kt == nk - 1) {
+                const int gr = row0 + wave * (BM / NW) + lane;
+                if (lane < BM / NW && gr < argM) {
+                    drow = p.row_map != nullptr ? p.row_map[gr] : gr;
+                    dval = p.row_len == nullptr || (gr % p.rows_per_item) < p.row_len[gr / p.rows_per_item];
+                }
+                if (p.bias != nullptr) {
+#pragma unroll
+                    for (int h = 0; h < BN / 64; ++h) bd[h] = p.bias[col0 + 64 * h + lane];
+                }
+            }
+        } else if (kt == nk - 1 && ksplit == 1) {
             if (p.bias != nullptr) bv = ld4(p.bias + col0 + ec);
             if (p.res != nullptr) {
 #pragma unroll
@@ -288,6 +351,22 @@
 #pragma unroll
     for (int e = 0; e < EI; ++e) reg_touch(rv[e]);
 
+    if constexpr (DIRECT) {
+        const int nout = pin_s(p.direct_cols);
+        for (int r = 0; r < BM / NW; ++r) {
+            const int d = __builtin_amdgcn_readlane(drow, r);
+            if (d < 0) continue;
+            const bool frame = __builtin_amdgcn_readlane(dval, r) != 0;
+            const float* src = ct + (wave * (BM / NW) + r) * CLD;
+            float* out = argY + (size_t)d * nout;
+#pragma unroll
+            for (int h = 0; h < BN / 64; ++h) {
+                const int col = col0 + 64 * h + lane;
+                if (col < nout) out[col] = frame ? (src[64 * h + lane] + bd[h]) + 0.f : 0.f;
+            }
+        }
+        return;
+    }
     if (ksplit > 1) {
         float* const Yz = argY + (size_t)kz * p.plane;
 #pragma unroll
@@ -317,7 +396,11 @@
 template <int BM, int BN>
 __global__ __launch_bounds__(256, 2) void gemm_big_split_kernel(const GemmArgs p) { gemm_big_split_body<BM, BN>(p); }
 template <int BM, int BN>
+__global__ __launch_bounds__(256, 2) void gemm_big_split_direct_kernel(const GemmArgs p) { gemm_big_split_body<BM, BN, true>(p); }
+template <int BM, int BN>
 __global__ __launch_bounds__(256, 2) void gemm_big_split_batch_kernel(const GemmBatch b) { gemm_big_split_body<BM, BN>(b.a[blockIdx.y]); }
+template <int BM, int BN>
+__global__ __launch_bounds__(256, 2) void gemm_big_split_agen_batch_kernel(const GemmBatch b) { gemm_big_split_body<BM, BN, false, true>(b.a[blockIdx.y]); }
 
 template <int BM, int BN, int WM, int WN, bool LN>
 __global__ __launch_bounds__(256) void gemm_big_kernel(const GemmArgs p) { gemm_big_body<BM, BN, WM, WN, LN>(p); }
@@ -344,6 +427,13 @@
 }
 
 bool gemm_big_supported(const GemmArgs& a) {
+    if (a.split && a.direct_cols > 0)
+        return a.M > 0 && a.K % 64 == 0 && a.K1 % 64 == 0 && a.N % 128 == 0 && a.lda % 4 == 0 && a.ldw % 4 == 0 && (!a.A2 || a.lda2 % 4 == 0) &&
+               a.direct_cols <= a.N && a.ldy == a.direct_cols && a.Y && !a.Ys && !a.res && a.act == ACT_NONE && a.ksplit <= 1 &&
+               (!a.row_len || a.rows_per_item > 0) && !a.ln_g && !a.mod && a.post_act == ACT_NONE;
+    if (a.direct_cols > 0) return false;
+    if (a.gen_nval != nullptr && !(a.split && a.K == 256 && a.A2 == nullptr && a.gen_beta && a.gen_mod && a.gen_B2 >= 0 && a.gen_stride % 4 == 0 && a.ksplit <= 1))
+        return false;
     if (a.split) return a.M > 0 && a.K % 64 == 0 && a.K1 % 64 == 0 && a.N % 128 == 0 && a.lda % 4 == 0 && a.ldw % 4 == 0 && (!a.A2 || a.lda2 % 4 == 0) &&
                         a.ldy % 64 == 0 && !a.ln_g && !a.mod && !a.row_len && !a.row_map && a.post_act == ACT_NONE && (a.Y || a.Ys);
     if (a.M < 4096 || a.K % BKB || a.K1 % BKB || (a.lda % 4) || (a.ldw % 4) || (a.A2 && (a.lda2 % 4))) return false;
@@ -353,11 +443,16 @@
 }
 
 int launch_gemm_big(const GemmArgs& a, hipStream_t s) {
+    if (a.gen_nval != nullptr) return LADIFF_ERR_ARG;
     if (a.split) {
         const int nbm = (a.M + 127) / 128, nbn = a.N / 128;
         const int ks = a.ksplit > 1 ? a.ksplit : 1;
         if (ks > 1 && ((a.K / 32) % ks != 0 || a.Y == nullptr || a.Ys != nullptr || a.plane == 0)) return LADIFF_ERR_ARG;
-        if (nbm * nbn <= 256 && a.M > 64) {
+        if (a.direct_cols > 0) {
+            const int nbm64 = (a.M + 63) / 64;
+            if (nbm * nbn <= 256 && a.M > 64) hipLaunchKernelGGL((gemm_big_split_direct_kernel<64, 128>), dim3(((nbm64 + 7) / 8) * 8 * nbn), dim3(256), 0, s, a);
+            else hipLaunchKernelGGL((gemm_big_split_direct_kernel<128, 128>), dim3(((nbm + 7) / 8) * 8 * nbn), dim3(256), 0, s, a);
+        } else if (nbm * nbn <= 256 && a.M > 64) {
             const int nbm64 = (a.M + 63) / 64;
             hipLaunchKernelGGL((gemm_big_split_kernel<64, 128>), dim3(((nbm64 + 7) / 8) * 8 * nbn, ks), dim3(256), 0, s, a);
         } else {
@@ -372,14 +467,17 @@
 }
 
 int launch_gemm_big_batch(const GemmBatch& b, int n, hipStream_t s) {
-    for (int i = 0; i < n; ++i) if (b.a[i].ksplit > 1) return LADIFF_ERR_ARG;
+    for (int i = 0; i < n; ++i) if (b.a[i].ksplit > 1 || b.a[i].direct_cols > 0) return LADIFF_ERR_ARG;
     if (b.a[0].split) {
         const GemmArgs& a = b.a[0];
         const int nbm = (a.M + 127) / 128, nbn = a.N / 128;
-        hipLaunchKernelGGL((gemm_big_split_batch_kernel<128, 128>), dim3(((nbm + 7) / 8) * 8 * nbn, n), dim3(256), 0, s, b);
+        for (int i = 0; i < n; ++i) if ((b.a[i].gen_nval != nullptr) != (a.gen_nval != nullptr)) return LADIFF_ERR_ARG;
+        if (a.gen_nval != nullptr) hipLaunchKernelGGL((gemm_big_split_agen_batch_kernel<128, 128>), dim3(((nbm + 7) / 8) * 8 * nbn, n), dim3(256), 0, s, b);
+        else hipLaunchKernelGGL((gemm_big_split_batch_kernel<128, 128>), dim3(((nbm + 7) / 8) * 8 * nbn, n), dim3(256), 0, s, b);
         LADIFF_LAUNCH_CHECK();
         return 0;
     }
+    if (b.a[0].gen_nval != nullptr) return LADIFF_ERR_ARG;
     if (b.a[0].ln_g != nullptr) return launch_big_batch<64, 256, 2, 2, true>(b, n, s);
     return launch_big_batch<128, 128, 2, 2, false>(b, n, s);
 }
diff --git a/ladiff_amd/csrc/graph_key.h b/ladiff_amd/csrc/graph_key.h
--- a/ladiff_amd/csrc/graph_key.h
+++ b/ladiff_amd/csrc/graph_key.h
@@ -119,9 +119,11 @@
     int fused_attn;
     int mlp_variant;
     int post_off;
+    int memory_operands;
 };
 constexpr int DEC_SMALL_ROWS = 4096;
-struct DecRoute { bool small, fused_attn, out_cross, fused_mlp, final_split, post; };
+constexpr int DEC_MEM_LAYER0 = 2, DEC_MEM_FINAL = 4;
+struct DecRoute { bool small, fused_attn, out_cross, fused_mlp, final_split, post, layer0_shared, final_direct; };
 inline DecRoute dec_route(bool split_mode, int rows, const DecSwitches& sw, int mlp_min_rows) {
     DecRoute r;
     r.small = split_mode && rows < DEC_SMALL_ROWS && sw.small_rows_path;
@@ -130,6 +132,8 @@
     r.fused_mlp = split_mode && sw.fused_mlp && (rows >= mlp_min_rows || sw.fused_mlp == 2);
     r.final_split = split_mode && rows >= DEC_SMALL_ROWS && sw.final_split;
     r.post = r.out_cross && r.fused_mlp && !r.small && !sw.post_off;
+    r.layer0_shared = r.post && !(sw.memory_operands & DEC_MEM_LAYER0);
+    r.final_direct = r.final_split && !(sw.memory_operands & DEC_MEM_FINAL);
     return r;
 }
 inline GraphKey decode_key(const float* const* w, const float* const* w_split, int n_params, uint64_t weights_generation, const float* z,
@@ -155,7 +159,7 @@
     k.add(sw.mlp_variant);
     k.add(sw.fused_attn);
     k.add(sw.out_cross);
-    k.add(sw.post_off);
+    k.add(sw.post_off | (sw.memory_operands << 8));
     k.add(weights_hash(w, w_split, n_params));
     k.add(weights_generation);
     return k;
diff --git a/ladiff_amd/csrc/kernels.h b/ladiff_amd/csrc/kernels.h
--- a/ladiff_amd/csrc/kernels.h
+++ b/ladiff_amd/csrc/kernels.h
@@ -37,6 +37,7 @@
 int launch_broadcast_pe(const float* pe, int B, int F, float* x, float* xs, hipStream_t s);
 int launch_broadcast_pe_ragged(const float* pe, const int32_t* row_off, int B, int F, int F_out, float* x, float* xs, int32_t* row_out,
                                hipStream_t s);
+int launch_dec_leader(const int32_t* lengths, const int32_t* row_off, int B, int F, int F_out, int32_t* leader, int32_t* row_out, hipStream_t s);
 int launch_relu(const float* x, float* y, size_t n, hipStream_t s);
 int launch_pad_rows(const float* src, const float* srcb, float* dst, float* dstb, int C, int Np, hipStream_t s);
 int launch_zero_fill(float* x, size_t n, hipStream_t s);
@@ -116,7 +117,8 @@
 int launch_self_attention(const float* qkv, const int32_t* lengths, const uint32_t* keybits, float* out, int B, int F, int nheads,
                           int causal, int split_out, hipStream_t s, const int32_t* row_off = nullptr);
 int launch_self_attention_split(const float* qkv, const int32_t* lengths, const uint32_t* keybits, float* out, int B, int F,
-                                 int nheads, int causal, int split_out, hipStream_t s, const int32_t* row_off = nullptr, int shared_qkv = 0);
+                                 int nheads, int causal, int split_out, hipStream_t s, const int32_t* row_off = nullptr, int shared_qkv = 0,
+                                 const int32_t* leader = nullptr);
 int launch_decoder_cross_attention(const float* q, const float* kv, const int32_t* counts, float* out, int B, int F,
                                    int T, int split_out, hipStream_t s);
 
diff --git a/ladiff_amd/csrc/model.h b/ladiff_amd/csrc/model.h
--- a/ladiff_amd/csrc/model.h
+++ b/ladiff_amd/csrc/model.h
@@ -15,6 +15,7 @@
                      size_t ws_floats, hipStream_t s, int b_lo = 0, int b_n = -1, int loop_mode = 0, int ntxt = 1,
                      const int32_t* d_base = nullptr, const float* dctab = nullptr);
 int denoiser_text_static(const DenoiserW& w, const float* text, int B2, float* cache, float* ws, size_t ws_floats, hipStream_t s);
+extern std::atomic<int> g_ctab_through_memory;
 int denoiser_ctab(const DenoiserW& w, const float* tables_lo, int n, float* cache, int B2, float* u, size_t u_floats, hipStream_t s,
                   const DenoiserW* w_split = nullptr);
 int linear_cross_attention(const DenoiserW& w, int layer, const float* x, const float* xf, const float* emb, const int32_t* counts,
@@ -31,8 +32,8 @@
 int diffusion_reverse(Sampler* sp, const DenoiserW& w, const DenoiserW* w_split, const ReverseArgs& a);
 
 struct DecSwitchAtoms {
-    std::atomic<int> fused_mlp{1}, small_rows_path{1}, final_split{1}, out_cross{1}, fused_attn{1}, mlp_variant{0}, post_off{0};
-    DecSwitches snapshot() const { return {fused_mlp, small_rows_path, final_split, out_cross, fused_attn, mlp_variant, post_off}; }
+    std::atomic<int> fused_mlp{1}, small_rows_path{1}, final_split{1}, out_cross{1}, fused_attn{1}, mlp_variant{0}, post_off{0}, memory_operands{0};
+    DecSwitches snapshot() const { return {fused_mlp, small_rows_path, final_split, out_cross, fused_attn, mlp_variant, post_off, memory_operands}; }
 };
 extern DecSwitchAtoms g_dec;
 int dec_mlp_prepare();
@@ -57,6 +58,7 @@
     const float *w1, *b1, *w2, *b2, *g3, *be3, *g4, *be4;
     float *y, *ys;
     int B, F, T, M;
+    const int32_t* leader = nullptr;
 };
 int dec_post_prepare();
 int launch_dec_post_gu(float* guws, size_t gu_layer, int n, int B, int T, hipStream_t s);
diff --git a/ladiff_amd/csrc/rowops.hip b/ladiff_amd/csrc/rowops.hip
--- a/ladiff_amd/csrc/rowops.hip
+++ b/ladiff_amd/csrc/rowops.hip
@@ -142,7 +142,7 @@
     const f32x4 sc = ld4(m + c), sh = ld4(m + 256 + c);
     f32x4 v = b < B2 ? ld4(nval + (size_t)b * D + c) : ld4(beta + c);
 #pragma unroll
-    for (int i = 0; i < 4; ++i) v[i] = silu(v[i] * (1.f + sc[i]) + sh[i]);
+    for (int i = 0; i < 4; ++i) v[i] = ca_table_value(v[i], sc[i], sh[i]);
     st4(u + (size_t)row * D + c, v);
 }
 __global__ __launch_bounds__(256) void ca_table_input_batch_kernel(const RowBatch rb, int step_stride, int B2, int M, int split_out) {
@@ -155,7 +155,7 @@
     const f32x4 sc = ld4(m + c), sh = ld4(m + 256 + c);
     f32x4 v = b < B2 ? ld4(rb.a[k] + (size_t)b * D + c) : ld4(rb.g[k] + c);
 #pragma unroll
-    for (int i = 0; i < 4; ++i) v[i] = silu(v[i] * (1.f + sc[i]) + sh[i]);
+    for (int i = 0; i < 4; ++i) v[i] = ca_table_value(v[i], sc[i], sh[i]);
     if (split_out) store_split4(rb.y[k] + (size_t)row * D, c, v);
     else st4(rb.y[k] + (size_t)row * D + c, v);
 }
@@ -234,6 +234,31 @@
 int launch_broadcast_pe(const float* pe, int B, int F, float* x, float* xs, hipStream_t s) {
     const int M = B * F;
     hipLaunchKernelGGL(broadcast_pe_kernel, dim3((M + ROWS_PER_BLOCK - 1) / ROWS_PER_BLOCK), dim3(256), 0, s, pe, F, M, x, xs);
+    LADIFF_LAUNCH_CHECK();
+    return 0;
+}
+
+__global__ __launch_bounds__(256) void dec_leader_kernel(const int32_t* __restrict__ lengths, const int32_t* __restrict__ row_off, int F,
+                                                         int F_out, int32_t* __restrict__ leader, int32_t* __restrict__ row_out) {
+    __shared__ int first;
+    const int b = blockIdx.x, t = threadIdx.x;
+    if (t == 0) first = b;
+    __syncthreads();
+    auto len_of = [&](int i) { const int l = lengths != nullptr ? lengths[i] : F; return l < 1 ? 1 : (l > F ? F : l); };
+    auto span_of = [&](int i) { return row_off != nullptr ? row_off[i + 1] - row_off[i] : F; };
+    const int len = len_of(b), span = span_of(b);
+    for (int i = t; i < b; i += 256)
+        if (len_of(i) == len && span_of(i) == span) { atomicMin(&first, i); break; }
+    __syncthreads();
+    if (t == 0) leader[b] = first;
+    if (row_off != nullptr) {
+        const int r0 = row_off[b];
+        for (int f = t; f < span && f < F; f += 256) row_out[(size_t)r0 + f] = b * F_out + f;
+    }
+}
+int launch_dec_leader(const int32_t* lengths, const int32_t* row_off, int B, int F, int F_out, int32_t* leader, int32_t* row_out, hipStream_t s) {
+    if (B == 0) return 0;
+    hipLaunchKernelGGL(dec_leader_kernel, dim3(B), dim3(256), 0, s, lengths, row_off, F, F_out, leader, row_out);
     LADIFF_LAUNCH_CHECK();
     return 0;
 }
```
